# philcn/DXRExperiments

Measured on AMD Instinct MI355X. Metric: Mrays/s (all traced rays: primary + secondary + shadow), 1080p 1 spp/frame progressive, rendered in deferred sets of 32 frames, higher is better.
Workload: dtype f32

## Files before the change

dxrexperiments_amd/csrc/rt_pipeline.hip:

```cpp
#include <hip/hip_fp16.h>

#include <array>
#include <new>
#include <utility>

#include "rt_shade.h"
#include "rt_pipeline_queues.h"

using namespace rtd;

namespace {

constexpr int CBLOCK = 1024;
RT_DEV void wave_add(uint32_t v, uint32_t *counter)
{
    for (int o = 32; o > 0; o >>= 1) v += (uint32_t)__shfl_xor((int)v, o, 64);
    if ((threadIdx.x & 63u) == 0u && v) atomicAdd(counter, v);
}


template <bool BATCH>
struct PrimarySrcT {
    const PipeDev &pd;
    RT_DEV uint32_t count() const { return pd.cap; }
    RT_DEV uint32_t flags() const { return RT_RAY_FLAG_CULL_BACK_FACING_TRIANGLES; }
    RT_DEV bool load(uint32_t q, RayD &r) const
    {
        uint32_t px, py;
        if (BATCH && pd.n_frames > 1u) {
            uint32_t ql;
            const uint32_t f = (uint32_t)__builtin_amdgcn_readfirstlane((int)slot_frame(pd, q, ql));
            const bool valid = pix_xy(pd, ql, px, py);
            r = primary_ray(pd, pd.pfcs[f].cameraParams, px, py);
            return valid;
        }
        const bool valid = pix_xy(pd, q, px, py);
        r = primary_ray(pd, px, py);
        return valid;
    }
    RT_DEV void overflow(uint32_t q) const
    {
        const uint32_t k = atomicAdd(&pd.retry[0], 1u);
        if (k < pd.retry_cap) pd.retry[2u + k] = q;
    }
};
typedef PrimarySrcT<true> PrimarySrc;
struct PrimaryRetrySrc {
    const PipeDev &pd;
    RT_DEV uint32_t count() const { const uint32_t n = pd.retry[0]; return n <= pd.retry_cap ? n : pd.cap; }
    RT_DEV uint32_t flags() const { return RT_RAY_FLAG_CULL_BACK_FACING_TRIANGLES; }
    RT_DEV bool load(uint32_t i, RayD &r, uint32_t &ticket) const
    {
        const uint32_t q = pd.retry[0] <= pd.retry_cap ? pd.retry[2u + i] : i;
        ticket = q;
        uint32_t px, py, ql;
        const uint32_t f = slot_frame(pd, q, ql);
        const bool valid = pix_xy(pd, ql, px, py);
        r = pd.n_frames > 1u ? primary_ray(pd, pd.pfcs[f].cameraParams, px, py) : primary_ray(pd, px, py);
        return valid;
    }
};
template <bool BATCH>
struct PrimarySinkT {
    const PipeDev &pd;
    RT_DEV void store(uint32_t q, const HitD &h, bool) const
    {
        const bool hit = h.inst != RT_NO_HIT;
        pd.lv[0].hit[q] = make_float4(hit ? h.t : HIT_MISS, h.u, h.v, __uint_as_float(h.prim));
        pd.lv[0].inst[q] = h.inst;
    }
};

#ifndef RT_WAVES_PER_EU
#define RT_WAVES_PER_EU __attribute__((amdgpu_waves_per_eu(TWO_LEVEL ? 5 : RT_ROWS(STACK) == RT_LDS_STACK_ROWS_SETS ? 7 : RT_ROWS(STACK) == RT_LDS_STACK_ROWS ? 6 : 1)))
#endif
template <int STACK, bool TWO_LEVEL, bool BATCH, bool PERSIST>
__global__ void __launch_bounds__(PBLOCK) RT_WAVES_PER_EU k_primary(PipeDev pd)
{
    __shared__ int smem[(RT_ROWS(STACK) + RT_TOP_ROWS(PBLOCK)) * PBLOCK];
    if (blockIdx.x == 0)
        for (uint32_t i = threadIdx.x; i < (uint32_t)(POOL_OFFSET_WORDS + POOL_BYTES / 4); i += PBLOCK) pd.counters[i] = 0u;
    PrimarySrcT<BATCH> src = {pd};
    PrimarySinkT<BATCH> sink = {pd};
    if (PERSIST) trace_wave<RT_ROWS(STACK), PBLOCK, TWO_LEVEL, 64u, false, false, false, RT_REFS(STACK)>(pd.sc, src, sink, pd.pools + POOL_BYTES / 4, smem, nullptr);
    else trace_wave<RT_ROWS(STACK), PBLOCK, TWO_LEVEL, 64u, false, false, true, RT_REFS(STACK)>(pd.sc, src, sink, nullptr, smem, nullptr);
}

template <int STACK, bool TWO_LEVEL>
__global__ void __launch_bounds__(PBLOCK) RT_WAVES_PER_EU k_primary_retry(PipeDev pd)
{
    __shared__ int smem[(RT_ROWS(STACK) + RT_TOP_ROWS(PBLOCK)) * PBLOCK];
    if (pd.retry[0] == 0u) return;
    PrimaryRetrySrc src = {pd};
    PrimarySinkT<true> sink = {pd};
    trace_wave<RT_ROWS(STACK), PBLOCK, TWO_LEVEL, 64u, false, false, false, RT_REFS(STACK)>(pd.sc, src, sink, nullptr, smem, nullptr);
}

constexpr int CTILES = 8;
__global__ void __launch_bounds__(CBLOCK) k_compact_level(PipeDev pd, int L)
{
    __shared__ uint32_t wave_total[CBLOCK / 64];
    __shared__ uint32_t block_base;
    uint32_t total_items, n = 0;
    if (L == 0) total_items = pd.cap;
    else { n = pd.counters[C_NHIT + L - 1]; total_items = (L == 1 ? 2u : 1u) * n; }
    if (L == 0 && pd.retry && blockIdx.x == 0 && threadIdx.x == 0) { pd.retry[1] = pd.retry[0]; pd.retry[0] = 0u; }
    const uint32_t first = blockIdx.x * (uint32_t)(CTILES * CBLOCK);
    if (first >= total_items) return;
    const uint32_t lane = threadIdx.x & 63u, wave = threadIdx.x >> 6;
    auto slot_of = [&](uint32_t idx) -> size_t { return L == 1 ? (size_t)(idx / n) * pd.lv[1].rstride + idx % n : (size_t)idx; };
    uint32_t flags = 0, mine = 0;
#pragma unroll 4
    for (int t = 0; t < CTILES; t++) {
        const uint32_t idx = first + (uint32_t)t * CBLOCK + threadIdx.x;
        const bool hit = idx < total_items && pd.lv[L].hit[slot_of(idx)].x >= 0.0f;
        flags |= (hit ? 1u : 0u) << t;
        mine += hit ? 1u : 0u;
    }
    for (int o = 32; o > 0; o >>= 1) mine += (uint32_t)__shfl_xor((int)mine, o, 64);
    if (lane == 0) wave_total[wave] = mine;
    __syncthreads();
    if (threadIdx.x == 0) {
        uint32_t sum = 0;
        for (int w = 0; w < CBLOCK / 64; w++) sum += wave_total[w];
        block_base = sum ? atomicAdd(&pd.counters[C_NHIT + L], sum) : 0u;
    }
    __syncthreads();
    uint32_t running = block_base;
    for (int t = 0; t < CTILES; t++) {
        const uint32_t idx = first + (uint32_t)t * CBLOCK + threadIdx.x;
        if (first + (uint32_t)t * CBLOCK >= total_items) break;
        const bool hit = (flags >> t) & 1u;
        const unsigned long long mask = __ballot(hit);
        __syncthreads();
        if (lane == 0) wave_total[wave] = (uint32_t)__popcll(mask);
        __syncthreads();
        uint32_t before = 0, tile_total = 0;
        for (int w = 0; w < CBLOCK / 64; w++) { const uint32_t c = wave_total[w]; before += w < (int)wave ? c : 0u; tile_total += c; }
        const uint32_t j = running + before + (uint32_t)__popcll(mask & ((1ull << lane) - 1ull));
        if (idx < total_items) {
            const size_t slot = slot_of(idx);
            pd.lv[L].slot_j[slot] = hit ? j : RT_NO_HIT;
            if (hit) pd.lv[L].jlist[j] = (uint32_t)slot;
        }
        running += tile_total;
    }
}

template <bool PRIMARY, bool BATCH, int LC>
RT_DEV void shade_emit_body(const PipeDev &pd_arg, int level, uint32_t shadow_slots, uint32_t emit_next)
{
    PipeDev pd = pd_arg;
    const int L = PRIMARY ? 0 : (LC >= 0 ? LC : level);
    __builtin_assume(PRIMARY || L >= 1);
    const uint32_t idx = blockIdx.x * PBLOCK + threadIdx.x;
    if (idx >= pd.counters[C_NHIT + L]) return;
    const uint32_t slot = pd.lv[L].jlist[idx];
    const uint32_t q = L == 0 ? slot : pd.lv[L].pix[slot];
    uint32_t px, py, ql = q, frame = 0;
    if (BATCH) { frame = slot_frame(pd, q, ql); pd.pfc = pd.pfcs[frame]; }
    (void)pix_xy(pd, ql, px, py);
    const RayD r = L == 0 ? primary_ray(pd, px, py) : load_ray(pd.lv[L].O, pd.lv[L].D, slot);
    const float4 h = pd.lv[L].hit[slot];
    if (!PRIMARY && !emit_next && pd.shadow_compact && !pd.skip_unlit) {
        const f3 P = r.o + r.d * h.x;
        uint32_t mask = 3u;
        if (pd.kind != RT_PIPELINE_REALTIME && pd.pfc.options.debug == 2) {
            uint32_t seed = init_rand(px + py * pd.width, pd.pfc.cameraParams.frameCount);
            mask = next_rand(seed) < 0.5f ? 1u : 2u;
        }
        if ((uint32_t)L < pd.sh_levels) pd.sh_hits[pd.sh_cbase[L] + idx] = make_float4(P.x, P.y, P.z, __uint_as_float(mask | (frame << 8)));
        return;
    }
    EmitIO io(pd, L, idx, q, frame);
    (void)closest_hit(pd, io, r, h.x, h.y, h.z, __float_as_uint(h.w), pd.lv[L].inst[slot], (uint32_t)L, px + py * pd.width);
    io.finish_shadows(shadow_slots);
    if (emit_next) {
        if (L == 0) {
            for (uint32_t w = 0; w < 2; w++)
                if (!(io.sec_mask & (1u << w))) store_invalid(pd.lv[1].O, pd.lv[1].D, (size_t)w * pd.lv[1].rstride + idx);
        } else if (L < MAXD && !io.sec_mask) store_invalid(pd.lv[L < MAXD ? L + 1 : MAXD].O, pd.lv[L < MAXD ? L + 1 : MAXD].D, idx);
    }
}
template <bool PRIMARY, bool BATCH>
__global__ void __launch_bounds__(PBLOCK) k_shade_emit(PipeDev pd, int level, uint32_t shadow_slots, uint32_t emit_next)
{
    if (PRIMARY || !BATCH) shade_emit_body<PRIMARY, BATCH, -1>(pd, level, shadow_slots, emit_next);
    else if (level == 1) shade_emit_body<PRIMARY, BATCH, 1>(pd, level, shadow_slots, emit_next);
    else if (level == 2) shade_emit_body<PRIMARY, BATCH, 2>(pd, level, shadow_slots, emit_next);
    else if (level == 3) shade_emit_body<PRIMARY, BATCH, 3>(pd, level, shadow_slots, emit_next);
    else shade_emit_body<PRIMARY, BATCH, MAXD>(pd, level, shadow_slots, emit_next);
}

struct QueueSrc {
    const float4 *O, *D;
    const uint32_t *count_ptr;
    uint32_t stride, batches, fl;
    RT_DEV uint32_t n() const { return *count_ptr; }
    RT_DEV uint32_t count() const { return n() * batches; }
    RT_DEV uint32_t flags() const { return fl; }
    RT_DEV size_t slot(uint32_t i) const
    {
        const uint32_t c = n(), b = i >= c ? 1u : 0u;
        return (size_t)b * stride + (i - b * c);
    }
    RT_DEV bool load(uint32_t i, RayD &r) const
    {
        const size_t sl = slot(i);
        const v4f a = ldg16(O, sl * 16), b = ldg16(D, sl * 16);
        r.o = mk3(a.x, a.y, a.z); r.tmin = a.w;
        r.d = mk3(b.x, b.y, b.z); r.tmax = b.w;
        return r.tmax > r.tmin;
    }
};
struct SecondarySink {
    QueueSrc q;
    float4 *hit1;
    uint32_t *inst1;
    RT_DEV void store(uint32_t i, const HitD &h, bool traced) const
    {
        const size_t sl = q.slot(i);
        const bool hit = h.inst != RT_NO_HIT;
        hit1[sl] = make_float4(hit ? h.t : (traced ? HIT_MISS : HIT_UNTRACED), h.u, h.v, __uint_as_float(h.prim));
        inst1[sl] = h.inst;
    }
};

struct ShadowQueue {
    const float4 *hits, *O, *D;
    uint32_t *vis;
    const uint32_t *nhit;
    uint32_t log2, fl;
    uint32_t lv_first, lv_count;
    uint32_t cbase[MAXD + 1], hstride[MAXD + 1];
    LightRays lights;
    const LightRays *frame_lights;
    ShadowCacheDev cache;
    RT_DEV uint32_t count() const
    {
        uint32_t b = 0;
#pragma unroll
        for (uint32_t k = 0; k <= (uint32_t)MAXD; k++) if (k >= lv_first && k < lv_first + lv_count) b += (nhit[k] + 63u) & ~63u;
        return b << log2;
    }
    RT_DEV uint32_t flags() const { return fl; }
};
template <bool BATCH>
struct ShadowSrcN : ShadowQueue {
    RT_DEV bool load(uint32_t i, RayD &r, uint32_t &ticket) const
    {
        uint32_t n = 0, R = 0, cb = 0, hs = 0, before = 0;
        ticket = 0;
#pragma unroll
        for (uint32_t k = 0; k <= (uint32_t)MAXD; k++) {
            if (k >= lv_first && k < lv_first + lv_count) {
                const uint32_t nk = nhit[k], Rk = (nk + 63u) & ~63u, start = before;
                before += Rk << log2;
                const bool here = i >= start;
                n = here ? nk : n; R = here ? Rk : R; cb = here ? cbase[k] : cb; hs = here ? hstride[k] : hs;
                if (here) ticket = start;
            }
        }
        const uint32_t local = i - ticket;
        uint32_t b = local >= R ? 1u : 0u;
        if (log2 > 1u) { b += local >= 2u * R ? 1u : 0u; b += local >= 3u * R ? 1u : 0u; }
        const uint32_t j = local - b * R;
        ticket = (cb << log2) + b * hs + j;
        r.o = mk3(0.0f, 0.0f, 0.0f);
        r.d = mk3(0.0f, 0.0f, 0.0f);
        r.tmin = 0.0f;
        r.tmax = -1.0f;
        if (j >= n) { ticket = RT_NO_HIT; return false; }
        if (lights.on) {
            const v4f a = ldg16(hits, (size_t)(cb + j) * 16);
            const uint32_t bits = __float_as_uint(a.w);
            r.o = mk3(a.x, a.y, a.z);
            if (!((bits >> b) & 1u)) return false;
            if ((bits >> (2u + b)) & 1u) { r.tmax = RT_TMAX_SKIPPED; return false; }
            r.tmin = RAY_EPSILON;
            const LightRays *per_frame = BATCH ? frame_lights : nullptr;
            if (per_frame) {
                const float *fl = b == 0u ? per_frame[(bits >> 8) & 0xffu].dir_to_light : per_frame[(bits >> 8) & 0xffu].point_pos;
                const f3 l = mk3(fl[0], fl[1], fl[2]);
                if (b == 0u) { r.d = l; r.tmax = RAY_MAX_T; }
                else {
                    const f3 path = l - r.o;
                    const float dist = length(path);
                    r.d = normalize(path);
                    r.tmax = dist - fmaxf(RAY_EPSILON, fl[3]);
                }
                return r.tmax > r.tmin;
            }
            if (b == 0u) {
                r.d = mk3(lights.dir_to_light[0], lights.dir_to_light[1], lights.dir_to_light[2]);
                r.tmax = RAY_MAX_T;
            } else {
                const f3 path = mk3(lights.point_pos[0], lights.point_pos[1], lights.point_pos[2]) - r.o;
                const float dist = length(path);
                r.d = normalize(path);
                r.tmax = dist - fmaxf(RAY_EPSILON, lights.point_free);
            }
            return r.tmax > r.tmin;
        }
        const v4f a = ldg16(O, (size_t)ticket * 16), d = ldg16(D, (size_t)ticket * 16);
        r.o = mk3(a.x, a.y, a.z); r.tmin = a.w;
        r.d = mk3(d.x, d.y, d.z); r.tmax = d.w;
        return r.tmax > r.tmin;
    }
    RT_DEV uint32_t cache_slot(const RayD &r) const
    {
        const uint32_t res = cache.res;
        if (!(r.tmax < 1.0e37f)) {
            float u = r.o.x * cache.ua[0] + r.o.y * cache.ua[1] + r.o.z * cache.ua[2] + cache.ua[3];
            float v = r.o.x * cache.va[0] + r.o.y * cache.va[1] + r.o.z * cache.va[2] + cache.va[3];
            u = fminf(fmaxf(u, 0.0f), cache.res_f - 1.0f);
            v = fminf(fmaxf(v, 0.0f), cache.res_f - 1.0f);
            return (uint32_t)u * res + (uint32_t)v;
        }
        const float mx = r.o.x - cache.lp[0], my = r.o.y - cache.lp[1], mz = r.o.z - cache.lp[2];
        const float ax = fabsf(mx), ay = fabsf(my), az = fabsf(mz);
        uint32_t face;
        float ma, s, t;
        if (ax >= ay && ax >= az) { face = mx < 0.0f ? 1u : 0u; ma = ax; s = my; t = mz; }
        else if (ay >= az) { face = my < 0.0f ? 3u : 2u; ma = ay; s = mz; t = mx; }
        else { face = mz < 0.0f ? 5u : 4u; ma = az; s = mx; t = my; }
        const float inv = __builtin_amdgcn_rcpf(ma), half = 0.5f * cache.res_f;
        const float cs = fminf(fmaxf((s * inv * 0.5f + 0.5f) * half, 0.0f), half - 1.0f);
        const float ct = fminf(fmaxf((t * inv * 0.5f + 0.5f) * half, 0.0f), half - 1.0f);
        const uint32_t r2 = res >> 1;
        return res * res + (face * r2 + (uint32_t)cs) * r2 + (uint32_t)ct;
    }
    static constexpr bool has_first_candidates = true;
    template <bool TWO_LEVEL>
    RT_DEV uint32_t cached_leaf(uint32_t ticket, const RayD &r, uint32_t &slot, uint32_t &instance) const
    {
        slot = RT_NO_HIT;
        instance = 0u;
        if (!cache.table) return RT_NO_HIT;
        slot = RT_NO_HIT;
        if (cache.px_base && ticket < 2u * cache.hstride0) {
            const uint32_t b = ticket >= cache.hstride0 ? 1u : 0u;
            uint32_t q = cache.jlist0[ticket - b * cache.hstride0];
            if (cache.n_frames > 1u) q = (__umulhi(q >> 6, cache.frames_magic) << 6) | (q & 63u);
            if (q < cache.px_slots) slot = cache.px_base + 2u * q + b;
        }
        if (slot == RT_NO_HIT) slot = cache_slot(r);
        if (TWO_LEVEL) {
            const uint2 e = ((const uint2 *)cache.table)[slot];
            instance = e.y;
            return e.x;
        }
        const uint32_t t = cache.table[slot];
        return t < cache.n_tris ? t : RT_NO_HIT;
    }
    template <bool TWO_LEVEL>
    RT_DEV void remember(uint32_t slot, uint32_t sorted_triangle, uint32_t instance) const
    {
        if (!cache.table || slot >= cache.entries) return;
        if (TWO_LEVEL) ((uint2 *)cache.table)[slot] = make_uint2(sorted_triangle, instance);
        else cache.table[slot] = sorted_triangle;
    }
};
struct ShadowSinkN {
    ShadowQueue s;
    RT_DEV void store(uint32_t ticket, const HitD &h, bool) const { if (ticket != RT_NO_HIT && h.inst == RT_NO_HIT) atomicOr(&s.vis[ticket >> 5], 1u << (ticket & 31u)); }
};

template <int STACK, bool TWO_LEVEL, bool BATCH>
__global__ void __launch_bounds__(PBLOCK) RT_WAVES_PER_EU k_trace_shadow(SceneDev sc, ShadowQueue queues, uint32_t *pool, uint32_t *stat)
{
    __shared__ int smem[(RT_ROWS(STACK) + RT_TOP_ROWS(PBLOCK)) * PBLOCK];
    ShadowSrcN<BATCH> src;
    static_cast<ShadowQueue &>(src) = queues;
    ShadowSinkN sink = {queues};
    trace_wave<RT_ROWS(STACK), PBLOCK, TWO_LEVEL, (!TWO_LEVEL && RT_ROWS(STACK) == RT_LDS_STACK_ROWS_SETS) ? RT_POOL_CHUNK_SETS_ANYHIT : RT_POOL_CHUNK, RT_SHADOW_UNORDERED != 0, false, false, RT_REFS(STACK)>(sc, src, sink, pool, smem, stat);
}

template <int STACK, bool TWO_LEVEL>
__global__ void __launch_bounds__(PBLOCK) RT_WAVES_PER_EU k_trace_secondary(SceneDev sc, QueueSrc src, float4 *hit1, uint32_t *inst1, uint32_t *pool, uint32_t *stat)
{
    __shared__ int smem[(RT_ROWS(STACK) + RT_TOP_ROWS(PBLOCK)) * PBLOCK];
    SecondarySink sink = {src, hit1, inst1};
    trace_wave<RT_ROWS(STACK), PBLOCK, TWO_LEVEL, (!TWO_LEVEL && RT_ROWS(STACK) == RT_LDS_STACK_ROWS_SETS) ? RT_POOL_CHUNK_SETS : RT_POOL_CHUNK, false, false, false, RT_REFS(STACK)>(sc, src, sink, pool, smem, stat);
}

struct NullSink { RT_DEV void store(uint32_t, const HitD &, bool) const {} };

template <bool TWO_LEVEL>
__global__ void __launch_bounds__(PBLOCK) k_walk_primary(PipeDev pd, unsigned long long *walk)
{
    __shared__ int smem[(RT_LDS_STACK_ROWS + RT_TOP_ROWS(PBLOCK)) * PBLOCK];
    PrimarySrc src = {pd};
    NullSink sink;
    trace_wave<RT_LDS_STACK_ROWS, PBLOCK, TWO_LEVEL, 64u, false, true, false, true>(pd.sc, src, sink, nullptr, smem, nullptr, walk);
}
template <bool TWO_LEVEL>
__global__ void __launch_bounds__(PBLOCK) k_walk_queue(SceneDev sc, QueueSrc src, unsigned long long *walk)
{
    __shared__ int smem[(RT_LDS_STACK_ROWS + RT_TOP_ROWS(PBLOCK)) * PBLOCK];
    NullSink sink;
    trace_wave<RT_LDS_STACK_ROWS, PBLOCK, TWO_LEVEL, RT_POOL_CHUNK, false, true, false, true>(sc, src, sink, nullptr, smem, nullptr, walk);
}
template <bool TWO_LEVEL>
__global__ void __launch_bounds__(PBLOCK) k_walk_shadow(SceneDev sc, ShadowQueue queue, unsigned long long *walk)
{
    __shared__ int smem[(RT_LDS_STACK_ROWS + RT_TOP_ROWS(PBLOCK)) * PBLOCK];
    ShadowSrcN<true> src;
    static_cast<ShadowQueue &>(src) = queue;
    NullSink sink;
    trace_wave<RT_LDS_STACK_ROWS, PBLOCK, TWO_LEVEL, RT_POOL_CHUNK, RT_SHADOW_UNORDERED != 0, true, false, true>(sc, src, sink, nullptr, smem, nullptr, walk);
}

RT_DEV void add_totals(const uint32_t *__restrict__ counters, unsigned long long *__restrict__ totals, uint32_t pixels, uint32_t frames)
{
    totals[0] += (unsigned long long)pixels * frames;
    totals[1] += counters[C_SECONDARY];
    totals[2] += counters[C_SHADOW] + counters[C_SHADOW_SKIPPED];
    totals[6] += counters[C_SHADOW_SKIPPED];
    totals[3] += counters[C_NHIT + 0];
    for (int l = 1; l <= MAXD; l++) totals[4] += counters[C_NHIT + l];
    totals[5] += frames;
}

RT_DEV float4 accumulate(const PipeDev &pd, const float4 prev, const Shaded &sh)
{
    const f3 c = sh.color;
    const float4 cur = make_float4(fmax2(c.x, 0.0f), fmax2(c.y, 0.0f), fmax2(c.z, 0.0f), 1.0f);
    if (pd.accum_mode == RT_ACCUM_SUM) return make_float4(prev.x + cur.x, prev.y + cur.y, prev.z + cur.z, prev.w + cur.w);
    const float n = (float)pd.pfc.cameraParams.accumCount;
    const float n1 = (float)(pd.pfc.cameraParams.accumCount + 1u);
    float4 m = make_float4((n * prev.x + cur.x) / n1, (n * prev.y + cur.y) / n1, (n * prev.z + cur.z) / n1, (n * prev.w + cur.w) / n1);
    if (pd.accum_f16 == 1u) m = make_float4(__half2float(__float2half_rn(m.x)), __half2float(__float2half_rn(m.y)), __half2float(__float2half_rn(m.z)), __half2float(__float2half_rn(m.w)));
    else if (pd.accum_f16 == 2u) m = make_float4(__half2float(__float2half_rz(m.x)), __half2float(__float2half_rz(m.y)), __half2float(__float2half_rz(m.z)), __half2float(__float2half_rz(m.w)));
    return m;
}
RT_DEV void write_aovs(const PipeDev &pd, size_t pixel, const Shaded &sh)
{
    pd.aov_direct[pixel] = make_float4(fmax2(sh.aov_direct.x, 0.0f), fmax2(sh.aov_direct.y, 0.0f), fmax2(sh.aov_direct.z, 0.0f), 1.0f);
    pd.aov_indirect[pixel] = make_float4(fmax2(sh.aov_indirect.x, 0.0f), fmax2(sh.aov_indirect.y, 0.0f), fmax2(sh.aov_indirect.z, 0.0f), 1.0f);
}

template <bool FLAT, bool BATCH>
__global__ void __launch_bounds__(PBLOCK) k_resolve(PipeDev pd_arg)
{
    PipeDev pd = pd_arg;
    const uint32_t ql = blockIdx.x * PBLOCK + threadIdx.x;
    if (ql == 0) add_totals(pd.counters, pd.totals, pd.n_pixels, pd.n_frames);
    if (ql >= pd.fcap) return;
    uint32_t px, py;
    if (!pix_xy(pd, ql, px, py)) return;
    const size_t pixel = (size_t)py * pd.width + px;
    const bool progressive = pd.kind != RT_PIPELINE_REALTIME;
#ifndef RT_RESOLVE_REG_ACC
#define RT_RESOLVE_REG_ACC 1
#endif
    constexpr bool KEEP = BATCH && !FLAT && RT_RESOLVE_REG_ACC;
    float4 acc = KEEP && progressive ? pd.accum[pixel] : make_float4(0.0f, 0.0f, 0.0f, 0.0f);
    for (uint32_t f = 0; f < (BATCH ? pd.n_frames : 1u); f++) {
        if (BATCH) pd.pfc = pd.pfcs[f];
        const uint32_t q = frame_slot(pd, f, ql);
        const RayD r = primary_ray(pd, px, py);
        const float4 h = pd.lv[0].hit[q];
        Shaded sh;
        if (h.x == HIT_MISS) {
            sh.color = sample_environment(pd, r.d);
            sh.aov_direct = sh.color;
            sh.aov_indirect = mk3(0.0f, 0.0f, 0.0f);
        } else if (FLAT) {
            LevelResolveIO io(pd, 0, pd.lv[0].slot_j[q]);
            sh = closest_hit_aov(pd, io, r, h.x, h.y, h.z, __float_as_uint(h.w), pd.lv[0].inst[q], 0u, px + py * pd.width);
        } else {
            ResolveIO<0, 1> io(pd, pd.lv[0].slot_j[q], px + py * pd.width);
            sh = closest_hit_aov(pd, io, r, h.x, h.y, h.z, __float_as_uint(h.w), pd.lv[0].inst[q], 0u, px + py * pd.width);
        }
        if (progressive) { acc = accumulate(pd, KEEP ? acc : pd.accum[pixel], sh); if (!KEEP) pd.accum[pixel] = acc; }
        else write_aovs(pd, pixel, sh);
    }
    if (KEEP && progressive) pd.accum[pixel] = acc;
}

template <bool BATCH, int LC>
RT_DEV void shade_level_body(const PipeDev &pd_arg, int level)
{
    PipeDev pd = pd_arg;
    const int L = LC >= 0 ? LC : level;
    const uint32_t idx = blockIdx.x * PBLOCK + threadIdx.x;
    if (idx >= pd.counters[C_NHIT + L]) return;
    const uint32_t slot = pd.lv[L].jlist[idx];
    const uint32_t q = pd.lv[L].pix[slot];
    uint32_t px, py, ql = q;
    if (BATCH) pd.pfc = pd.pfcs[slot_frame(pd, q, ql)];
    (void)pix_xy(pd, ql, px, py);
    const RayD r = load_ray(pd.lv[L].O, pd.lv[L].D, slot);
    const float4 h = pd.lv[L].hit[slot];
    LevelResolveIO io(pd, L, idx);
    const f3 c = closest_hit(pd, io, r, h.x, h.y, h.z, __float_as_uint(h.w), pd.lv[L].inst[slot], (uint32_t)L, px + py * pd.width);
    pd.lv[L].color[slot] = make_float4(c.x, c.y, c.z, 0.0f);
}
template <bool BATCH>
__global__ void __launch_bounds__(PBLOCK) k_shade_level(PipeDev pd, int L)
{
    if (!BATCH) shade_level_body<BATCH, -1>(pd, L);
    else if (L == 1) shade_level_body<BATCH, 1>(pd, L);
    else if (L == 2) shade_level_body<BATCH, 2>(pd, L);
    else if (L == 3) shade_level_body<BATCH, 3>(pd, L);
    else shade_level_body<BATCH, MAXD>(pd, L);
}

RT_DEV void wave_add64(unsigned long long v, unsigned long long *counter)
{
    for (int o = 32; o > 0; o >>= 1) v += (unsigned long long)__shfl_xor((long long)v, o, 64);
    if ((threadIdx.x & 63u) == 0u && v) atomicAdd(counter, v);
}

template <class Src>
__global__ void __launch_bounds__(PBLOCK)
k_count_queue(SceneDev sc, Src src, unsigned long long *__restrict__ out)
{
    const uint32_t idx = blockIdx.x * PBLOCK + threadIdx.x;
    unsigned long long rays = 0, nodes = 0, tris = 0;
    if (idx < src.count()) {
        RayD r;
        uint32_t ticket;
        if (load_ray_of(src, idx, r, ticket, 0)) {
            uint32_t cn, ct;
            (void)trace_canonical(sc, r, src.flags(), cn, ct);
            rays = 1; nodes = cn; tris = ct;
        }
    }
    wave_add64(rays, &out[0]);
    wave_add64(nodes, &out[1]);
    wave_add64(tris, &out[2]);
}

__global__ void __launch_bounds__(PBLOCK) k_count_primary(PipeDev pd, unsigned long long *__restrict__ out)
{
    const uint32_t q = blockIdx.x * PBLOCK + threadIdx.x;
    unsigned long long rays = 0, nodes = 0, tris = 0;
    RayD r;
    const PrimarySrc src = {pd};
    if (q < pd.cap && src.load(q, r)) {
        uint32_t cn, ct;
        (void)trace_canonical(pd.sc, r, RT_RAY_FLAG_CULL_BACK_FACING_TRIANGLES, cn, ct);
        rays = 1; nodes = cn; tris = ct;
    }
    wave_add64(rays, &out[0]);
    wave_add64(nodes, &out[1]);
    wave_add64(tris, &out[2]);
}

__global__ void k_debug_cube(PipeDev pd, const float *__restrict__ dirs, float *__restrict__ out, size_t n)
{
    const size_t i = (size_t)blockIdx.x * blockDim.x + threadIdx.x;
    if (i >= n) return;
    const f3 c = sample_cube(pd, mk3(dirs[3 * i], dirs[3 * i + 1], dirs[3 * i + 2]));
    out[3 * i] = c.x; out[3 * i + 1] = c.y; out[3 * i + 2] = c.z;
}


}

namespace {

template <int STACK, bool TWO_LEVEL>
int launch_frame(rt_pipeline *p, PipeDev &pd, uint32_t shadow_slots, bool counted)
{
    hipError_t first_error = hipSuccess;
    auto record = [&](hipEvent_t e, hipStream_t s) { const hipError_t rc = hipEventRecord(e, s); if (first_error == hipSuccess) first_error = rc; };
    hipStream_t st = p->ctx->stream;
    const bool T = p->ring_frames > 0;
    const size_t ring_slot = T ? (size_t)(p->ring_pos % (uint64_t)p->ring_frames) : 0;
    hipEvent_t *ev = T ? &p->ring[ring_slot * EV_COUNT] : nullptr;
    const uint32_t cap = pd.cap;
    rt_context *ctx = p->ctx;
    const uint32_t levels = frame_levels(p);
    const bool deep = levels > 1, compact = pd.shadow_compact != 0;
    const uint32_t any = RT_RAY_FLAG_ACCEPT_FIRST_HIT_AND_END_SEARCH | RT_RAY_FLAG_SKIP_CLOSEST_HIT_SHADER;
    size_t hits_l = cap, slots = cap;
    size_t sh_total = 0;
    auto size_next = [&](uint32_t l, bool casts_shadows, bool spawns) -> int {
        if (counted) {
            HIP_TRY(hipMemcpyAsync(ctx->pinned, &pd.counters[C_NHIT + l], 4, hipMemcpyDeviceToHost, st));
            HIP_TRY(hipStreamSynchronize(st));
            hits_l = round64((size_t)ctx->pinned[0]);
            if (hits_l == 0) hits_l = 64;
        } else hits_l = l == 0 ? (size_t)cap : 2 * (size_t)cap;
        if (hits_l > 0xffffffc0ull / 2) { rt_set_error("render: more than 2^31 hits at radiance level %u", l); return RT_ERR_UNSUPPORTED; }
        pd.lv[l].hstride = (uint32_t)hits_l;
        if (casts_shadows) {
            if (((sh_total + hits_l) << pd.sh_log2) >= 0xffffffc0ull) { rt_set_error("render: more than 2^32 shadow rays in one set of launches"); return RT_ERR_UNSUPPORTED; }
            if (counted) RT_TRY(reserve_shadows(p, sh_total + hits_l, pd.sh_log2, compact, sh_total));
            pd.sh_cbase[l] = (uint32_t)sh_total;
            sh_total += hits_l;
        }
        bind_level(p, pd, (int)l);
        if (spawns) {
            slots = (l == 0 ? 2 : 1) * hits_l;
            if (l == 0) pd.lv[1].rstride = (uint32_t)hits_l;
            if (counted) RT_TRY(reserve_level_rays(p, l + 1, slots, deep));
            bind_level(p, pd, (int)l + 1);
        }
        return RT_OK;
    };
    if (T) record(ev[0], st);
    if (pd.primary_persistent) HIP_TRY(hipMemsetAsync(pd.pools + POOL_BYTES / 4, 0, PRIMARY_POOL_WORDS * 4, st));
    if (pd.primary_persistent) {
        if (pd.n_frames > 1u) k_primary<STACK, TWO_LEVEL, true, true><<<rt_persistent_grid(ctx, k_primary<STACK, TWO_LEVEL, true, true>, PBLOCK, cap), PBLOCK, 0, st>>>(pd);
        else k_primary<STACK, TWO_LEVEL, false, true><<<rt_persistent_grid(ctx, k_primary<STACK, TWO_LEVEL, false, true>, PBLOCK, cap), PBLOCK, 0, st>>>(pd);
    } else {
        if (pd.n_frames > 1u) k_primary<STACK, TWO_LEVEL, true, false><<<blocks(cap), PBLOCK, 0, st>>>(pd);
        else k_primary<STACK, TWO_LEVEL, false, false><<<blocks(cap), PBLOCK, 0, st>>>(pd);
        if (pd.retry) k_primary_retry<STACK, TWO_LEVEL><<<rt_persistent_grid(ctx, k_primary_retry<STACK, TWO_LEVEL>, PBLOCK, cap), PBLOCK, 0, st>>>(pd);
    }
    k_compact_level<<<(cap + CTILES * CBLOCK - 1) / (CTILES * CBLOCK), CBLOCK, 0, st>>>(pd, 0);
    if (T) record(ev[1], st);
    RT_TRY(size_next(0, true, levels >= 1));
    const bool B = pd.n_frames > 1u;
    if (B) k_shade_emit<true, true><<<blocks(hits_l), PBLOCK, 0, st>>>(pd, 0, shadow_slots, levels >= 1 ? 1u : 0u);
    else k_shade_emit<true, false><<<blocks(hits_l), PBLOCK, 0, st>>>(pd, 0, shadow_slots, levels >= 1 ? 1u : 0u);
    if (T) record(ev[2], st);
    const LightRays lr = light_rays(pd);
    for (uint32_t l = 1; l <= levels; l++) {
        const QueueSrc rays = {pd.lv[l].O, pd.lv[l].D, &pd.counters[C_NHIT + l - 1], pd.lv[1].rstride, l == 1 ? 2u : 1u, RT_RAY_FLAG_NONE};
        k_trace_secondary<STACK, TWO_LEVEL><<<rt_persistent_grid(ctx, k_trace_secondary<STACK, TWO_LEVEL>, PBLOCK, slots), PBLOCK, 0, st>>>(
            pd.sc, rays, pd.lv[l].hit, pd.lv[l].inst, pd.pools + (size_t)l * RT_POOL_GROUPS * RT_POOL_STRIDE, &pd.counters[C_SECONDARY]);
        k_compact_level<<<(unsigned)((slots + CTILES * CBLOCK - 1) / (CTILES * CBLOCK)), CBLOCK, 0, st>>>(pd, (int)l);
        if (T) record(ev[3 + 2 * (l - 1)], st);
        const bool casts_shadows = l < pd.sh_levels, spawns = l < levels;
        RT_TRY(size_next(l, casts_shadows, spawns));
        if (casts_shadows || spawns) {
            if (B) k_shade_emit<false, true><<<blocks(hits_l), PBLOCK, 0, st>>>(pd, (int)l, 2u, spawns ? 1u : 0u);
            else k_shade_emit<false, false><<<blocks(hits_l), PBLOCK, 0, st>>>(pd, (int)l, 2u, spawns ? 1u : 0u);
        }
        if (T) record(ev[4 + 2 * (l - 1)], st);
    }
    {
        ShadowQueue sq;
        memset(&sq, 0, sizeof sq);
        sq.hits = pd.sh_hits; sq.O = pd.sh_O; sq.D = pd.sh_D; sq.vis = pd.sh_vis;
        sq.nhit = &pd.counters[C_NHIT];
        sq.log2 = pd.sh_log2; sq.fl = any;
        sq.lv_first = 0; sq.lv_count = pd.sh_levels;
        for (int k = 0; k <= MAXD; k++) { sq.cbase[k] = pd.sh_cbase[k]; sq.hstride[k] = pd.lv[k].hstride; }
        sq.lights = lr;
        sq.frame_lights = B ? pd.frame_lights : nullptr;
        sq.cache = p->shadow_cache_dev;
        sq.cache.jlist0 = pd.lv[0].jlist;
        sq.cache.hstride0 = pd.lv[0].hstride;
        sq.cache.n_frames = pd.n_frames;
        sq.cache.frames_magic = (uint32_t)(0x100000000ull / (pd.n_frames ? pd.n_frames : 1u)) + 1u;
        if (sq.cache.px_slots > pd.fcap) sq.cache.px_slots = pd.fcap;
        const size_t rays_max = sh_total << pd.sh_log2;
        HIP_TRY(hipMemsetAsync(pd.sh_vis, 0, ((rays_max + 31) / 32) * 4, st));
        if (B) k_trace_shadow<STACK, TWO_LEVEL, true><<<rt_persistent_grid(ctx, k_trace_shadow<STACK, TWO_LEVEL, true>, PBLOCK, rays_max), PBLOCK, 0, st>>>(
            pd.sc, sq, pd.pools, &pd.counters[C_SHADOW]);
        else k_trace_shadow<STACK, TWO_LEVEL, false><<<rt_persistent_grid(ctx, k_trace_shadow<STACK, TWO_LEVEL, false>, PBLOCK, rays_max), PBLOCK, 0, st>>>(
            pd.sc, sq, pd.pools, &pd.counters[C_SHADOW]);
    }
    if (T) record(ev[EV_SHADOW], st);
    if (levels <= 1) {
        if (B) k_resolve<false, true><<<blocks(pd.fcap), PBLOCK, 0, st>>>(pd);
        else k_resolve<false, false><<<blocks(pd.fcap), PBLOCK, 0, st>>>(pd);
    } else {
        for (uint32_t l = levels; l >= 1; l--) {
            const size_t n_l = pd.lv[l].hstride;
            if (B) k_shade_level<true><<<blocks(n_l), PBLOCK, 0, st>>>(pd, (int)l);
            else k_shade_level<false><<<blocks(n_l), PBLOCK, 0, st>>>(pd, (int)l);
        }
        if (B) k_resolve<true, true><<<blocks(pd.fcap), PBLOCK, 0, st>>>(pd);
        else k_resolve<true, false><<<blocks(pd.fcap), PBLOCK, 0, st>>>(pd);
    }
    if (T) { record(ev[EV_RESOLVE], st); p->ring_levels[ring_slot] = (uint8_t)levels; p->ring_nframes[ring_slot] = (uint8_t)pd.n_frames; p->ring_pos++; }
    HIP_TRY(first_error);
    return RT_OK;
}

template <int STACK>
int launch_frame_any(rt_pipeline *p, PipeDev &pd, uint32_t shadow_slots, bool counted)
{
    if (p->scene->has_refs)
        return p->scene->two_level ? launch_frame<STACK + RT_STACK_REFS, true>(p, pd, shadow_slots, counted) : launch_frame<STACK + RT_STACK_REFS, false>(p, pd, shadow_slots, counted);
    return p->scene->two_level ? launch_frame<STACK, true>(p, pd, shadow_slots, counted) : launch_frame<STACK, false>(p, pd, shadow_slots, counted);
}

template <bool TWO_LEVEL>
static int count_walk_launch(rt_pipeline *p, unsigned long long *w)
{
    hipStream_t st = p->ctx->stream;
    const rt_context *ctx = p->ctx;
    const PipeDev &pd = p->last_pd;
    const uint32_t cap = pd.cap;
    const uint32_t any = RT_RAY_FLAG_ACCEPT_FIRST_HIT_AND_END_SEARCH | RT_RAY_FLAG_SKIP_CLOSEST_HIT_SHADER;
    k_walk_primary<TWO_LEVEL><<<rt_persistent_grid(ctx, k_walk_primary<TWO_LEVEL>, PBLOCK, cap), PBLOCK, 0, st>>>(pd, w + RT_WALK_WORDS * RT_STAGE_PRIMARY);
    const unsigned gq = rt_persistent_grid(ctx, k_walk_queue<TWO_LEVEL>, PBLOCK, (size_t)cap * 2);
    const unsigned gs = rt_persistent_grid(ctx, k_walk_shadow<TWO_LEVEL>, PBLOCK, (size_t)cap * 2);
    ShadowQueue sq;
    memset(&sq, 0, sizeof sq);
    sq.hits = pd.sh_hits; sq.O = pd.sh_O; sq.D = pd.sh_D; sq.vis = pd.sh_vis;
    sq.nhit = &pd.counters[C_NHIT];
    sq.log2 = pd.sh_log2; sq.fl = any;
    sq.lights = light_rays(pd);
    sq.frame_lights = pd.n_frames > 1u ? pd.frame_lights : nullptr;
    for (int k = 0; k <= MAXD; k++) { sq.cbase[k] = pd.sh_cbase[k]; sq.hstride[k] = pd.lv[k].hstride; }
    sq.lv_first = 0; sq.lv_count = 1;
    k_walk_shadow<TWO_LEVEL><<<gs, PBLOCK, 0, st>>>(pd.sc, sq, w + RT_WALK_WORDS * RT_STAGE_SHADOW0);
    const uint32_t levels = pd.max_rad < (uint32_t)MAXD ? pd.max_rad : (uint32_t)MAXD;
    for (uint32_t l = 1; l <= levels; l++)
        k_walk_queue<TWO_LEVEL><<<gq, PBLOCK, 0, st>>>(pd.sc, QueueSrc{pd.lv[l].O, pd.lv[l].D, &pd.counters[C_NHIT + l - 1], pd.lv[1].rstride, l == 1 ? 2u : 1u, RT_RAY_FLAG_NONE},
                                                       w + RT_WALK_WORDS * RT_STAGE_SECONDARY);
    if (pd.sh_levels > 1u) {
        sq.lv_first = 1; sq.lv_count = pd.sh_levels - 1u;
        k_walk_shadow<TWO_LEVEL><<<gs, PBLOCK, 0, st>>>(pd.sc, sq, w + RT_WALK_WORDS * RT_STAGE_SHADOW1);
    }
    HIP_TRY(hipGetLastError());
    return RT_OK;
}

}

int rt_frame_launch(rt_pipeline *p, PipeDev &pd, uint32_t shadow_slots, bool counted, bool set_rows)
{
    if (p->ctx->lds_stack_rows == RT_LDS_STACK_ROWS_TEST) return launch_frame_any<RT_LDS_STACK_ROWS_TEST>(p, pd, shadow_slots, counted);
    if (set_rows) return launch_frame<RT_LDS_STACK_ROWS_SETS, false>(p, pd, shadow_slots, counted);
    return launch_frame_any<RT_LDS_STACK_ROWS>(p, pd, shadow_slots, counted);
}

int rt_frame_count_walk(rt_pipeline *p, unsigned long long *w)
{
    return p->scene->two_level ? count_walk_launch<true>(p, w) : count_walk_launch<false>(p, w);
}

int rt_frame_count_work(rt_pipeline *p, unsigned long long *w)
{
    hipStream_t st = p->ctx->stream;
    const PipeDev &pd = p->last_pd;
    const uint32_t cap = pd.cap;
    const uint32_t any = RT_RAY_FLAG_ACCEPT_FIRST_HIT_AND_END_SEARCH | RT_RAY_FLAG_SKIP_CLOSEST_HIT_SHADER;
    k_count_primary<<<blocks(cap), PBLOCK, 0, st>>>(pd, w + 3 * RT_STAGE_PRIMARY);
    ShadowSrcN<true> sq;
    memset(&sq, 0, sizeof sq);
    sq.hits = pd.sh_hits; sq.O = pd.sh_O; sq.D = pd.sh_D; sq.vis = pd.sh_vis;
    sq.nhit = &pd.counters[C_NHIT];
    sq.log2 = pd.sh_log2; sq.fl = any;
    sq.lights = light_rays(pd);
    sq.frame_lights = pd.n_frames > 1u ? pd.frame_lights : nullptr;
    for (int k = 0; k <= MAXD; k++) { sq.cbase[k] = pd.sh_cbase[k]; sq.hstride[k] = pd.lv[k].hstride; }
    sq.lv_first = 0; sq.lv_count = 1;
    k_count_queue<<<blocks((size_t)pd.lv[0].hstride << pd.sh_log2), PBLOCK, 0, st>>>(pd.sc, sq, w + 3 * RT_STAGE_SHADOW0);
    const uint32_t levels = pd.max_rad < (uint32_t)MAXD ? pd.max_rad : (uint32_t)MAXD;
    size_t deeper = 0;
    for (uint32_t l = 1; l <= levels; l++) {
        const uint32_t batches = l == 1 ? 2u : 1u;
        const size_t slots = l == 1 ? 2 * (size_t)pd.lv[1].rstride : (size_t)pd.lv[l - 1].hstride;
        k_count_queue<<<blocks(slots), PBLOCK, 0, st>>>(pd.sc, QueueSrc{pd.lv[l].O, pd.lv[l].D, &pd.counters[C_NHIT + l - 1], pd.lv[1].rstride, batches, RT_RAY_FLAG_NONE},
                                                        w + 3 * RT_STAGE_SECONDARY);
        if (l < pd.sh_levels) deeper += pd.lv[l].hstride;
    }
    if (pd.sh_levels > 1u) {
        sq.lv_first = 1; sq.lv_count = pd.sh_levels - 1u;
        k_count_queue<<<blocks(deeper << pd.sh_log2), PBLOCK, 0, st>>>(pd.sc, sq, w + 3 * RT_STAGE_SHADOW1);
    }
    HIP_TRY(hipGetLastError());
    return RT_OK;
}

int rt_frame_debug_cube(hipStream_t st, const PipeDev &pd, const float *dirs, float *out, size_t n)
{
    k_debug_cube<<<blocks(n), PBLOCK, 0, st>>>(pd, dirs, out, n);
    HIP_TRY(hipGetLastError());
    return RT_OK;
}
```

dxrexperiments_amd/csrc/rt_pipeline_dev.h:

```cpp
#pragma once

#include "rt_trace_wave.h"

namespace rtp {

using namespace rtd;


constexpr int PBLOCK = 256;
#ifndef RT_SHADOW_UNORDERED
#define RT_SHADOW_UNORDERED 1
#endif
static_assert(RT_SHADOW_UNORDERED != 0, "the shadow stage counts skipped slots in the ANYHIT walk only");

#define RAY_MAX_T 1.0e+38f
#define RAY_EPSILON 0.0001f
#define HLSL_PI 3.1415927f

#define HIT_MISS -1.0f
#define HIT_UNTRACED -2.0f

constexpr int MAXD = 4;
enum { C_NHIT = 0,
       C_SECONDARY = MAXD + 1, C_SHADOW = MAXD + 2,
       C_SHADOW_SKIPPED = MAXD + 3,
       C_COUNT = MAXD + 4 };

struct LevelDev {
    uint32_t rstride;
    uint32_t hstride;
    float4 *O, *D;
    float4 *hit; uint32_t *inst;
    uint32_t *slot_j, *jlist;
    uint32_t *pix;
    float4 *color;
};

struct LightRays {
    uint32_t on;
    float dir_to_light[3];
    float point_pos[3];
    float point_free;
};

struct ShadowCacheDev {
    uint32_t *table;
    float ua[4], va[4];
    float lp[3];
    float res_f;
    uint32_t res;
    uint32_t two_level;
    uint32_t n_tris;
    uint32_t px_base, entries;
    const uint32_t *jlist0;
    uint32_t hstride0;
    uint32_t n_frames, frames_magic;
    uint32_t px_slots;
};

#define RT_MAX_BATCH 32u

struct PipeDev {
    SceneDev sc;
    rt_per_frame_constants pfc;
    uint32_t n_frames, fcap;
    const rt_per_frame_constants *pfcs;
    const LightRays *frame_lights;
    const rt_material_params *mats;
    uint32_t nmats;
    const float4 *env;
    uint32_t env_size;
    uint32_t env_filter;
    float env_const[3];
    uint32_t width, height;
    uint32_t x0, y0, tw, th, cap;
    uint32_t tiles_x;
    uint32_t band_rows, band_rank, band_world;
    uint32_t n_pixels;
    uint32_t max_rad, max_shadow;
    uint32_t accum_mode;
    uint32_t accum_f16;
    uint32_t skip_unlit;
    uint32_t shadow_compact;
    uint32_t kind;
    uint32_t primary_persistent;
    float4 *accum;
    float4 *aov_direct, *aov_indirect;
    uint32_t *counters;
    uint32_t *retry;
    uint32_t retry_cap;
    unsigned long long *totals;
    float point_free;
    float4 *sh_hits, *sh_O, *sh_D;
    uint32_t *sh_vis;
    uint32_t sh_log2;
    uint32_t sh_levels;
    uint32_t sh_cbase[MAXD + 1];
    uint32_t *pools;
    LevelDev lv[MAXD + 1];
};

constexpr size_t POOL_BYTES = (size_t)(1 + MAXD) * RT_POOL_GROUPS * RT_POOL_STRIDE * 4;
constexpr size_t PRIMARY_POOL_WORDS = (size_t)RT_POOL_GROUPS * RT_POOL_STRIDE;
constexpr size_t POOL_OFFSET_WORDS = 64;

RT_DEV size_t sh_ray(const PipeDev &pd, int L, uint32_t idx, uint32_t s)
{
    return ((size_t)pd.sh_cbase[L] << pd.sh_log2) + (size_t)s * pd.lv[L].hstride + idx;
}
RT_DEV uint32_t shadow_bit(const PipeDev &pd, size_t n)
{
    return (pd.sh_vis[n >> 5] >> (uint32_t)(n & 31u)) & 1u;
}

inline unsigned blocks(size_t n) { return (unsigned)((n + PBLOCK - 1) / PBLOCK); }

}

using namespace rtp;


struct rt_pipeline {
    rt_context *ctx = nullptr;
    uint32_t kind = RT_PIPELINE_PROGRESSIVE;
    DevBuf aov_own;
    rt_scene *scene = nullptr;
    std::vector<rt_material_params> mats;
    DevBuf d_mats;
    bool mats_dirty = true;
    DevBuf d_env;
    uint32_t env_size = 0;
    uint32_t env_filter = RT_CUBE_SEAMLESS;
    float env_const[3] = {0.5f, 0.5f, 0.5f};
    uint32_t width = 0, height = 0, format = RT_FORMAT_R32G32B32A32_FLOAT;
    DevBuf accum_own;
    float4 *accum = nullptr;
    rt_per_frame_constants pfc;
    bool have_pfc = false;
    uint32_t max_rad = 1, max_shadow = 2, accum_mode = RT_ACCUM_RUNNING_MEAN, accum_f16 = 0;
    uint32_t skip_unlit = 0;
    size_t queue_budget = 0;
    bool counted_queues = false;
    uint32_t deferred_max = 0;
    std::vector<rt_per_frame_constants> pending;
    int deferred_error = RT_OK;
    std::string deferred_error_msg;
    struct LevelBuf { DevBuf O, D, hit, inst, slot_j, jlist, pix, color; } lv[MAXD + 1];
    DevBuf sh_hits, sh_O, sh_D, sh_vis;
    DevBuf counters;
    DevBuf retry;
    DevBuf half_out;
    std::vector<hipEvent_t> ring;
    std::vector<uint8_t> ring_levels;
    std::vector<uint8_t> ring_nframes;
    DevBuf batch_consts;
    int ring_frames = 0;
    DevBuf shadow_cache;
    int shadow_cache_res = -1;
    uint32_t shadow_cache_gen = 0xffffffffu;
    float shadow_cache_centre[3] = {0, 0, 0}, shadow_cache_radius = 1.0f;
    ShadowCacheDev shadow_cache_dev = {};
    struct FreeSphere {
        DevBuf d_min;
        float *h_min = nullptr;
        hipEvent_t landed = nullptr;
        uint32_t asked_gen = 0xffffffffu, known_gen = 0xffffffffu;
        float asked_lp[3] = {0, 0, 0}, known_lp[3] = {0, 0, 0}, known_radius = 0.0f;
        float asked_size = 0.0f;
        bool in_flight = false;
    } free_sphere;
    struct PrimaryMode {
        uint32_t *h_count = nullptr;
        hipEvent_t landed = nullptr;
        bool in_flight = false;
        uint32_t asked_slots = 0;
        uint32_t gen = 0xffffffffu;
        int samples = 0;
        bool persistent = false;
    } primary_mode;
    uint64_t ring_pos = 0;
    DevBuf totals, work;
    PipeDev last_pd;
    rt_stats stats;
    uint32_t last_tile[4] = {0, 0, 0, 0};
    uint32_t last_pixels = 0;
    bool rendered = false;
    uint32_t last_scene_gen = 0;
};

int rt_pipeline_flush_pending(rt_pipeline *p);

namespace rtp {


constexpr int EV_COUNT = 5 + 2 * MAXD;
constexpr int EV_SHADOW = 3 + 2 * MAXD, EV_RESOLVE = 4 + 2 * MAXD;

}
```

dxrexperiments_amd/csrc/rt_pipeline_render.hip:

```cpp
#include <hip/hip_fp16.h>

#include <array>
#include <new>
#include <utility>

#include "rt_pipeline_queues.h"

using namespace rtd;

namespace {

__global__ void __launch_bounds__(PBLOCK) k_free_sphere(SceneDev sc, uint32_t two_level, uint32_t n, float lx, float ly, float lz, uint32_t *out_bits)
{
    const uint32_t i = blockIdx.x * PBLOCK + threadIdx.x;
    float d2 = __uint_as_float(0x7f800000u);
    if (i < n) {
        float lo[3], hi[3];
        if (two_level) {
            const InstanceRec &in = sc.inst[i];
            for (int c = 0; c < 3; c++) { lo[c] = in.wlo[c]; hi[c] = in.whi[c]; }
        } else {
            const TriRec t = sc.inst[0].tris[i];
            const float vx[3] = {t.a.x, t.a.w, t.b.z}, vy[3] = {t.a.y, t.b.x, t.b.w}, vz[3] = {t.a.z, t.b.y, t.c.x};
            lo[0] = fminf(vx[0], fminf(vx[1], vx[2])); hi[0] = fmaxf(vx[0], fmaxf(vx[1], vx[2]));
            lo[1] = fminf(vy[0], fminf(vy[1], vy[2])); hi[1] = fmaxf(vy[0], fmaxf(vy[1], vy[2]));
            lo[2] = fminf(vz[0], fminf(vz[1], vz[2])); hi[2] = fmaxf(vz[0], fmaxf(vz[1], vz[2]));
        }
        const float l[3] = {lx, ly, lz};
        float s = 0.0f;
        bool known = true;
        for (int c = 0; c < 3; c++) {
            const float d = l[c] < lo[c] ? lo[c] - l[c] : l[c] > hi[c] ? l[c] - hi[c] : 0.0f;
            known = known && lo[c] == lo[c] && hi[c] == hi[c];
            s += d * d;
        }
        d2 = known ? s : 0.0f;
    }
    for (int o = 32; o > 0; o >>= 1) d2 = fminf(d2, __shfl_xor(d2, o, 64));
    if ((threadIdx.x & 63u) == 0u) atomicMin(out_bits, __float_as_uint(d2));
}

void free_sphere_poll(rt_pipeline::FreeSphere &f)
{
    if (f.in_flight && hipEventQuery(f.landed) == hipSuccess) {
        f.in_flight = false;
        f.known_gen = f.asked_gen;
        memcpy(f.known_lp, f.asked_lp, sizeof f.known_lp);
        double size = 0.0;
        for (int c = 0; c < 3; c++) size = fmax(size, fmax(fabs((double)f.asked_lp[c]), (double)f.asked_size));
        const double r = sqrt((double)*f.h_min) * 0.99 - (double)RAY_EPSILON - size * 4e-6;
        f.known_radius = r > 0.0 && r < 1e30 ? (float)r : 0.0f;
    }
}

float free_radius(rt_pipeline *p, const PipeDev &pd, const float lp[3])
{
    rt_pipeline::FreeSphere &f = p->free_sphere;
    const rt_scene *s = p->scene;
    hipStream_t st = p->ctx->stream;
    if (!(lp[0] == lp[0] && lp[1] == lp[1] && lp[2] == lp[2])) return 0.0f;
    if (!f.h_min) {
        if (hipHostMalloc((void **)&f.h_min, 64, hipHostMallocDefault) != hipSuccess) { f.h_min = nullptr; return 0.0f; }
        if (hipEventCreateWithFlags(&f.landed, hipEventDisableTiming) != hipSuccess || f.d_min.reserve(64) != RT_OK) return 0.0f;
    }
    free_sphere_poll(f);
    const bool known = f.known_gen == s->generation && memcmp(f.known_lp, lp, sizeof f.known_lp) == 0;
    const bool asked = f.in_flight && f.asked_gen == s->generation && memcmp(f.asked_lp, lp, sizeof f.asked_lp) == 0;
    if (!known && !asked && !f.in_flight) {
        const uint32_t n = s->two_level ? (uint32_t)s->inst.size() : (s->inst.empty() || !s->inst[0].model ? 0u : s->inst[0].model->n_recs);
        if (n == 0u || !f.landed) return 0.0f;
        if (hipMemsetD32Async((hipDeviceptr_t)f.d_min.p, 0x7f800000, 1, st) != hipSuccess) return 0.0f;
        k_free_sphere<<<(n + PBLOCK - 1) / PBLOCK, PBLOCK, 0, st>>>(pd.sc, s->two_level ? 1u : 0u, n, lp[0], lp[1], lp[2], f.d_min.as<uint32_t>());
        if (hipMemcpyAsync(f.h_min, f.d_min.p, 4, hipMemcpyDeviceToHost, st) != hipSuccess || hipEventRecord(f.landed, st) != hipSuccess) return 0.0f;
        f.in_flight = true;
        f.asked_gen = s->generation;
        const float *bb = s->two_level ? s->tlas.bounds : s->inst[0].model->blas.bounds;
        f.asked_size = 0.0f;
        for (int c = 0; c < 6; c++) f.asked_size = bb[c] == bb[c] ? fmaxf(f.asked_size, fabsf(bb[c])) : __builtin_inff();
        memcpy(f.asked_lp, lp, sizeof f.asked_lp);
    }
    return known ? f.known_radius : 0.0f;
}

int prepare_shadow_cache(rt_pipeline *p, const rt_per_frame_constants &pfc, const LightRays &lr)
{
    p->shadow_cache_dev = ShadowCacheDev{};
    const rt_scene *s = p->scene;
    if (p->shadow_cache_res == 0 || s->inst.empty()) return RT_OK;
    size_t n_tris_all = 0;
    for (const SceneInstance &si : s->inst) {
        if (!si.model || si.model->n_tris >= (1u << 28)) return RT_OK;
        n_tris_all += si.model->n_tris;
    }
    int want = p->shadow_cache_res;
    if (want < 0) {
        want = p->ctx->opt_shadow_cache_res;
        if (want == 0) return RT_OK;
    }
    if (want < 0) {
        const double target = 8.0 * sqrt((double)n_tris_all);
        want = 1024;
        while (want < 8192 && (double)want < target) want *= 2;
    }
    if (want > 8192) want = 8192;
    if (want < 16) want = 16;
    const uint32_t res = (uint32_t)want & ~1u;
    const int per_pixel_opt = p->ctx->opt_shadow_cache_pixels;
    const bool per_pixel = per_pixel_opt < 0 ? s->two_level : per_pixel_opt != 0;
    const size_t cells = (size_t)res * res + 6u * (size_t)(res / 2) * (res / 2);
    const size_t px_slots = per_pixel ? (size_t)((p->width + 7u) / 8u) * ((p->height + 7u) / 8u) * 64u : 0;
    const size_t entries = cells + 2 * px_slots, entry_bytes = s->two_level ? 8 : 4;
    if (entries >= 0xffffffffull) return RT_OK;
    if (p->shadow_cache.bytes < entries * entry_bytes) { RT_TRY(p->shadow_cache.reserve(entries * entry_bytes)); p->shadow_cache_gen = 0xffffffffu; }
    if (lr.on == 0xffffffffu) return RT_OK;
    if (p->shadow_cache_gen != s->generation) {
        HIP_TRY(hipMemsetAsync(p->shadow_cache.p, 0xff, entries * entry_bytes, p->ctx->stream));
        const float *bb = s->two_level ? s->tlas.bounds : s->inst[0].model->blas.bounds;
        float lo[3], hi[3];
        for (int c = 0; c < 3; c++) {
            lo[c] = bb[c]; hi[c] = bb[3 + c];
            if (!(lo[c] > -1e30f && hi[c] < 1e30f && lo[c] <= hi[c])) { lo[c] = -1.0f; hi[c] = 1.0f; }
        }
        float r2 = 0.0f;
        for (int c = 0; c < 3; c++) { p->shadow_cache_centre[c] = 0.5f * (lo[c] + hi[c]); const float h = 0.5f * (hi[c] - lo[c]); r2 += h * h; }
        p->shadow_cache_radius = r2 > 0.0f && r2 < 1e30f ? sqrtf(r2) : 1.0f;
        p->shadow_cache_gen = s->generation;
    }
    ShadowCacheDev c = {};
    c.table = p->shadow_cache.as<uint32_t>();
    c.res = res; c.res_f = (float)res;
    c.two_level = s->two_level ? 1u : 0u;
    c.n_tris = s->two_level ? 0u : s->inst[0].model->n_recs;
    c.entries = (uint32_t)entries;
    c.px_base = px_slots ? (uint32_t)cells : 0u;
    c.px_slots = (uint32_t)px_slots;
    const float d[3] = {lr.dir_to_light[0], lr.dir_to_light[1], lr.dir_to_light[2]};
    const float ref[3] = {fabsf(d[1]) < 0.9f ? 0.0f : 1.0f, fabsf(d[1]) < 0.9f ? 1.0f : 0.0f, 0.0f};
    float a[3] = {d[1] * ref[2] - d[2] * ref[1], d[2] * ref[0] - d[0] * ref[2], d[0] * ref[1] - d[1] * ref[0]};
    const float al = sqrtf(a[0] * a[0] + a[1] * a[1] + a[2] * a[2]);
    if (!(al > 1e-6f)) { a[0] = 1.0f; a[1] = 0.0f; a[2] = 0.0f; } else { a[0] /= al; a[1] /= al; a[2] /= al; }
    const float b[3] = {d[1] * a[2] - d[2] * a[1], d[2] * a[0] - d[0] * a[2], d[0] * a[1] - d[1] * a[0]};
    const float k = 0.5f * (float)res / p->shadow_cache_radius;
    c.ua[3] = 0.5f * (float)res; c.va[3] = 0.5f * (float)res;
    for (int i = 0; i < 3; i++) {
        c.ua[i] = a[i] * k; c.va[i] = b[i] * k;
        c.ua[3] -= p->shadow_cache_centre[i] * c.ua[i];
        c.va[3] -= p->shadow_cache_centre[i] * c.va[i];
        c.lp[i] = lr.point_pos[i];
    }
    (void)pfc;
    p->shadow_cache_dev = c;
    return RT_OK;
}

int scene_for_set(rt_pipeline *p, uint32_t n_frames, size_t cap, SceneDev *out, bool *sets_kernels = nullptr)
{
    rt_context *ctx = p->ctx;
    const bool seven_waves_always = ctx->opt_seven_waves_always;
    const bool set_rows = (n_frames > 1 || seven_waves_always) && !p->scene->two_level && !p->scene->has_refs && ctx->lds_stack_rows != RT_LDS_STACK_ROWS_TEST && RT_LDS_STACK_ROWS_SETS != RT_LDS_STACK_ROWS;
    const size_t resident = (size_t)ctx->cu_count * (ctx->blocks_per_cu_override > (uint32_t)RT_RESIDENT_BLOCKS_PER_CU ? ctx->blocks_per_cu_override : (uint32_t)RT_RESIDENT_BLOCKS_PER_CU) * PBLOCK;
    (void)cap;
    if (sets_kernels) *sets_kernels = set_rows;
    return rt_scene_dev_for_launch(ctx, p->scene, set_rows ? RT_LDS_STACK_ROWS_SETS : rt_lds_stack_rows(ctx), resident, out);
}

}

extern "C" {

static int render_region(rt_pipeline *p, uint32_t width, uint32_t height, uint32_t x0, uint32_t y0, uint32_t x1, uint32_t y1,
                         uint32_t band_rows, uint32_t band_rank, uint32_t band_world, const rt_per_frame_constants *frames = nullptr, uint32_t n_frames = 1)
{
    RT_REQUIRE(p, "null pipeline");
    if (!p->scene || !p->scene->built) { rt_set_error("render: acceleration structures not built"); return RT_ERR_STATE; }
    if (!p->accum) { rt_set_error("render: no output resource"); return RT_ERR_STATE; }
    if (!frames && !p->have_pfc) { rt_set_error("render: update() has not been called"); return RT_ERR_STATE; }
    if (!frames) { frames = &p->pfc; n_frames = 1; }
    RT_REQUIRE(n_frames >= 1 && n_frames <= RT_MAX_BATCH, "batch size");
    if (p->mats.empty()) { rt_set_error("render: no material"); return RT_ERR_STATE; }
    RT_REQUIRE(width == p->width && height == p->height, "width/height differ from the output resource");
    if (x1 > width) x1 = width;
    if (!band_rows && y1 > height) y1 = height;
    RT_REQUIRE(x0 < x1 && y0 < y1, "empty tile");
    rt_context *ctx = p->ctx;
    HIP_TRY(hipSetDevice(ctx->device));
    hipStream_t st = ctx->stream;
    p->rendered = false;
    if (p->kind == RT_PIPELINE_PROGRESSIVE && frames[0].cameraParams.accumCount >= frames[0].options.maxIterations) {
        memset(&p->stats, 0, sizeof p->stats);
        return RT_OK;
    }
    if (p->mats_dirty) {
        RT_TRY(p->d_mats.reserve(sizeof(rt_material_params) * p->mats.size()));
        HIP_TRY(hipMemcpyAsync(p->d_mats.p, p->mats.data(), sizeof(rt_material_params) * p->mats.size(), hipMemcpyHostToDevice, st));
        p->mats_dirty = false;
    }
    const uint32_t tw = x1 - x0, th = y1 - y0;
    const uint32_t tiles_x = (tw + 7u) / 8u, fcap = tiles_x * ((th + 7u) / 8u) * 64u;
    RT_REQUIRE((uint64_t)fcap * n_frames < 0x40000000ull, "batch: more than 2^30 pixel slots in one set of launches");
    const uint32_t cap = fcap * n_frames;
    const bool ao_view = p->kind == RT_PIPELINE_PROGRESSIVE && frames[0].options.showAmbientOcclusionOnly;
    const uint32_t shadow_slots = ao_view ? 4u : 2u;
    const uint32_t levels_now = frame_levels(p);
    const bool counted = worst_case_queue_bytes(cap, levels_now, p->max_shadow, shadow_slots, !ao_view) > queue_budget(p);
    if (p->counters.bytes < POOL_OFFSET_WORDS * 4 + POOL_BYTES + PRIMARY_POOL_WORDS * 4) {
        RT_TRY(p->counters.reserve(POOL_OFFSET_WORDS * 4 + POOL_BYTES + PRIMARY_POOL_WORDS * 4));
        HIP_TRY(hipMemsetAsync(p->counters.p, 0, p->counters.bytes, st));
    }
    if (counted) RT_TRY(reserve_level_rays(p, 0, cap, levels_now > 1));
    else RT_TRY(reserve_worst_case(p, cap, levels_now, p->max_shadow, shadow_slots, !ao_view));
    p->counted_queues = counted;
    if (!p->totals.p) {
        RT_TRY(p->totals.reserve(8 * sizeof(unsigned long long)));
        HIP_TRY(hipMemsetAsync(p->totals.p, 0, 8 * sizeof(unsigned long long), st));
    }
    PipeDev pd;
    bool set_rows = false;
    RT_TRY(scene_for_set(p, n_frames, cap, &pd.sc, &set_rows));
    pd.pfc = frames[0];
    pd.n_frames = n_frames; pd.fcap = fcap;
    pd.pfcs = nullptr; pd.frame_lights = nullptr;
    pd.shadow_compact = ao_view ? 0u : 1u;
    const bool free_on = ctx->opt_free_radius;
    {
        const float lp0[3] = {frames[0].pointLight.worldPos.x, frames[0].pointLight.worldPos.y, frames[0].pointLight.worldPos.z};
        pd.point_free = free_on ? free_radius(p, pd, lp0) : 0.0f;
    }
    if (ao_view) p->shadow_cache_dev = ShadowCacheDev{};
    else RT_TRY(prepare_shadow_cache(p, frames[0], light_rays(1u, frames[0])));
    if (n_frames > 1) {
        const size_t cb = sizeof(rt_per_frame_constants) * RT_MAX_BATCH, lb = sizeof(LightRays) * RT_MAX_BATCH;
        RT_TRY(p->batch_consts.reserve(cb + lb));
        std::vector<unsigned char> stage(cb + lb, 0);
        for (uint32_t f = 0; f < n_frames; f++) {
            memcpy(&stage[sizeof(rt_per_frame_constants) * f], &frames[f], sizeof(rt_per_frame_constants));
            LightRays lr = light_rays(pd.shadow_compact, frames[f]);
            lr.point_free = free_on && memcmp(lr.point_pos, &frames[0].pointLight.worldPos, 3 * sizeof(float)) == 0 ? pd.point_free : 0.0f;
            memcpy(&stage[cb + sizeof(LightRays) * f], &lr, sizeof lr);
        }
        HIP_TRY(hipMemcpyAsync(p->batch_consts.p, stage.data(), cb + lb, hipMemcpyHostToDevice, st));
        pd.pfcs = p->batch_consts.as<rt_per_frame_constants>();
        pd.frame_lights = (const LightRays *)((const char *)p->batch_consts.p + cb);
    }
    pd.mats = p->d_mats.as<rt_material_params>();
    pd.nmats = (uint32_t)p->mats.size();
    pd.env = p->d_env.as<float4>();
    pd.env_size = p->env_size;
    pd.env_filter = p->env_filter;
    for (int k = 0; k < 3; k++) pd.env_const[k] = p->env_const[k];
    pd.width = width; pd.height = height;
    pd.x0 = x0; pd.y0 = y0; pd.tw = tw; pd.th = th; pd.cap = cap; pd.tiles_x = tiles_x;
    pd.band_rows = band_rows; pd.band_rank = band_rank; pd.band_world = band_world;
    uint32_t owned_rows = th;
    if (band_rows) {
        owned_rows = 0;
        for (uint32_t b = band_rank; (uint64_t)b * band_rows < height; b += band_world)
            owned_rows += (uint64_t)(b + 1) * band_rows <= height ? band_rows : height - b * band_rows;
    }
    pd.n_pixels = tw * owned_rows;
    pd.max_rad = p->max_rad; pd.max_shadow = p->max_shadow;
    pd.sh_log2 = ao_view ? 2u : 1u;
    pd.sh_levels = shadow_levels(levels_now, p->max_shadow);
    for (int k = 0; k <= MAXD; k++) pd.sh_cbase[k] = 0;
    pd.accum_mode = p->accum_mode;
    pd.accum_f16 = p->accum_f16;
    pd.skip_unlit = p->skip_unlit;
    pd.kind = p->kind;
    {
        rt_pipeline::PrimaryMode &pm = p->primary_mode;
        if (pm.gen != p->scene->generation) { pm.gen = p->scene->generation; pm.samples = 0; pm.persistent = false; pm.in_flight = false; }
        if (pm.in_flight && hipEventQuery(pm.landed) == hipSuccess) {
            pm.in_flight = false;
            pm.samples++;
            if ((double)*pm.h_count > 0.002 * (double)pm.asked_slots) pm.persistent = true;
        }
        pd.primary_persistent = (ctx->opt_primary_persistent < 0 ? (p->scene->two_level || pm.persistent) : ctx->opt_primary_persistent != 0) ? 1u : 0u;
    }
    pd.retry = nullptr;
    pd.retry_cap = 0;
    if (pd.sc.deep_stack && !pd.primary_persistent) {
        const uint32_t want = ctx->opt_primary_retry_cap ? ctx->opt_primary_retry_cap : (1u << 20);
        if (p->retry.bytes < (2 + (size_t)want) * 4) {
            RT_TRY(p->retry.reserve((2 + (size_t)want) * 4));
            HIP_TRY(hipMemsetAsync(p->retry.p, 0, 8, st));
        }
        pd.retry = p->retry.as<uint32_t>();
        pd.retry_cap = want;
    }
    pd.accum = p->accum;
    pd.aov_direct = p->accum;
    pd.aov_indirect = p->aov_own.as<float4>();
    pd.counters = p->counters.as<uint32_t>();
    for (int l = 0; l <= MAXD; l++) {
        bind_level(p, pd, l);
        pd.lv[l].rstride = cap;
        pd.lv[l].hstride = l == 0 ? cap : 2u * cap;
    }
    static_assert(C_COUNT <= POOL_OFFSET_WORDS, "scalar counters overlap the chunk pools");
    pd.pools = pd.counters + POOL_OFFSET_WORDS;
    pd.totals = p->totals.as<unsigned long long>();
    RT_TRY(rt_frame_launch(p, pd, shadow_slots, counted, set_rows));
    HIP_TRY(hipGetLastError());
    if (pd.retry && !p->primary_mode.in_flight && p->primary_mode.samples < 8 && ctx->opt_primary_persistent < 0) {
        rt_pipeline::PrimaryMode &pm = p->primary_mode;
        if (!pm.h_count) {
            if (hipHostMalloc((void **)&pm.h_count, 64, hipHostMallocDefault) != hipSuccess) pm.h_count = nullptr;
            else if (hipEventCreateWithFlags(&pm.landed, hipEventDisableTiming) != hipSuccess) { (void)hipHostFree(pm.h_count); pm.h_count = nullptr; pm.landed = nullptr; }
        }
        if (pm.h_count && hipMemcpyAsync(pm.h_count, pd.retry + 1, 4, hipMemcpyDeviceToHost, st) == hipSuccess && hipEventRecord(pm.landed, st) == hipSuccess) {
            pm.in_flight = true;
            pm.asked_slots = cap;
        }
    }
    p->last_pd = pd;
    p->last_scene_gen = p->scene->generation;
    p->last_tile[0] = x0; p->last_tile[1] = y0; p->last_tile[2] = x1; p->last_tile[3] = y1;
    p->last_pixels = pd.n_pixels * n_frames;
    p->rendered = true;
    return RT_OK;
}

static int render_frames(rt_pipeline *p, uint32_t width, uint32_t height, const rt_per_frame_constants *constants, uint32_t n,
                         uint32_t band_rows, uint32_t band_rank, uint32_t band_world)
{
    uint32_t band_count = 0;
    if (band_rows) {
        RT_TRY(rt_tile_bands(height, band_rows, band_rank, band_world, nullptr, nullptr, 0, &band_count));
        if (band_count == 0) n = 0;
    }
    uint32_t batch_max = RT_MAX_BATCH;
    if (p->ctx->opt_batch_max >= 1 && p->ctx->opt_batch_max <= RT_MAX_BATCH) batch_max = p->ctx->opt_batch_max;
    std::vector<rt_per_frame_constants> run;
    auto flush = [&]() -> int {
        for (size_t at = 0; at < run.size();) {
            const size_t n_now = run.size() - at < batch_max ? run.size() - at : batch_max;
            const int rc = band_rows ? render_region(p, width, height, 0, 0, width, band_count * band_rows, band_rows, band_rank, band_world, run.data() + at, (uint32_t)n_now)
                                     : render_region(p, width, height, 0, 0, width, height, 0, 0, 1, run.data() + at, (uint32_t)n_now);
            if (rc == RT_ERR_OOM && n_now > 1) { batch_max = (uint32_t)(n_now / 2); continue; }
            if (rc != RT_OK) { run.clear(); return rc; }
            at += n_now;
        }
        run.clear();
        return RT_OK;
    };
    for (uint32_t i = 0; i < n; i++) {
        const rt_per_frame_constants &c = constants[i];
        if (c.cameraParams.accumCount >= c.options.maxIterations) continue;
        if (!run.empty() && (run.size() >= batch_max || (run[0].options.showAmbientOcclusionOnly != 0) != (c.options.showAmbientOcclusionOnly != 0))) RT_TRY(flush());
        run.push_back(c);
    }
    return flush();
}

}

static int flush_pending_now(rt_pipeline *p)
{
    if (p->pending.empty()) return RT_OK;
    std::vector<rt_per_frame_constants> frames;
    frames.swap(p->pending);
    std::vector<rt_pipeline *> &reg = p->ctx->deferred;
    for (size_t k = 0; k < reg.size(); k++) if (reg[k] == p) { reg.erase(reg.begin() + (long)k); break; }
    const rt_per_frame_constants keep = p->pfc;
    const int rc = render_frames(p, p->width, p->height, frames.data(), (uint32_t)frames.size(), 0, 0, 1);
    p->pfc = keep;
    return rc;
}

int rt_pipeline_flush_pending(rt_pipeline *p)
{
    if (!p) return RT_OK;
    if (p->deferred_error != RT_OK) {
        const int rc = p->deferred_error;
        rt_set_error("deferred frames were lost: %s", p->deferred_error_msg.c_str());
        p->deferred_error = RT_OK;
        p->deferred_error_msg.clear();
        return rc;
    }
    return flush_pending_now(p);
}

int rt_context_flush_deferred(rt_context *ctx)
{
    if (!ctx) return RT_OK;
    while (!ctx->deferred.empty()) {
        rt_pipeline *p = ctx->deferred.back();
        const int rc = flush_pending_now(p);
        if (rc != RT_OK && p->deferred_error == RT_OK) { p->deferred_error = rc; p->deferred_error_msg = rt_last_error(); }
    }
    return RT_OK;
}

extern "C" {

int rt_pipeline_flush(rt_pipeline *p)
{
    RT_REQUIRE(p, "null pipeline");
    return rt_pipeline_flush_pending(p);
}

int rt_pipeline_set_deferred(rt_pipeline *p, uint32_t max_frames)
{
    RT_REQUIRE(p, "null pipeline");
    RT_REQUIRE(max_frames <= RT_MAX_BATCH, "set_deferred: at most 32 frames share a set of launches");
    RT_REQUIRE(p->kind == RT_PIPELINE_PROGRESSIVE || max_frames <= 1, "set_deferred: only the progressive pipeline accumulates frames");
    RT_TRY(rt_pipeline_flush_pending(p));
    p->deferred_max = max_frames;
    return RT_OK;
}

int rt_pipeline_get_deferred(const rt_pipeline *p, uint32_t *max_frames, uint32_t *pending)
{
    RT_REQUIRE(p, "null pipeline");
    if (max_frames) *max_frames = p->deferred_max;
    if (pending) *pending = (uint32_t)p->pending.size();
    return RT_OK;
}

int rt_pipeline_render_tile(rt_pipeline *p, uint32_t width, uint32_t height, uint32_t x0, uint32_t y0, uint32_t x1, uint32_t y1)
{
    RT_TRY(rt_pipeline_flush_pending(p));
    return render_region(p, width, height, x0, y0, x1, y1, 0, 0, 1);
}

int rt_pipeline_render_bands(rt_pipeline *p, uint32_t width, uint32_t height, uint32_t band_rows, uint32_t rank, uint32_t world)
{
    RT_REQUIRE(world > 0 && rank < world, "rank outside [0, world)");
    RT_REQUIRE(band_rows > 0 && band_rows % 8 == 0, "band_rows must be a positive multiple of 8 (pixel slots are 8x8 tiles)");
    RT_TRY(rt_pipeline_flush_pending(p));
    uint32_t n = 0;
    RT_TRY(rt_tile_bands(height, band_rows, rank, world, nullptr, nullptr, 0, &n));
    if (n == 0) return RT_OK;
    return render_region(p, width, height, 0, 0, width, n * band_rows, band_rows, rank, world);
}

int rt_pipeline_render(rt_pipeline *p, uint32_t width, uint32_t height)
{
    RT_REQUIRE(p, "null pipeline");
    if (p->deferred_max > 1 && p->kind == RT_PIPELINE_PROGRESSIVE) {
        if (!p->scene || !p->scene->built) { rt_set_error("render: acceleration structures not built"); return RT_ERR_STATE; }
        if (!p->accum) { rt_set_error("render: no output resource"); return RT_ERR_STATE; }
        if (!p->have_pfc) { rt_set_error("render: update() has not been called"); return RT_ERR_STATE; }
        if (p->mats.empty()) { rt_set_error("render: no material"); return RT_ERR_STATE; }
        RT_REQUIRE(width == p->width && height == p->height, "width/height differ from the output resource");
        if (p->pending.empty()) p->ctx->deferred.push_back(p);
        p->pending.push_back(p->pfc);
        p->rendered = false;
        if (p->pending.size() >= p->deferred_max) return rt_pipeline_flush_pending(p);
        return RT_OK;
    }
    return rt_pipeline_render_tile(p, width, height, 0, 0, width, height);
}

int rt_pipeline_render_batch(rt_pipeline *p, uint32_t width, uint32_t height, const rt_per_frame_constants *constants, uint32_t n)
{
    RT_REQUIRE(p && (constants || n == 0), "null argument");
    RT_REQUIRE(p->kind == RT_PIPELINE_PROGRESSIVE, "render_batch: only the progressive pipeline accumulates frames");
    RT_TRY(rt_pipeline_flush_pending(p));
    RT_TRY(render_frames(p, width, height, constants, n, 0, 0, 1));
    if (n) { p->pfc = constants[n - 1]; p->have_pfc = true; }
    return RT_OK;
}

int rt_pipeline_render_bands_batch(rt_pipeline *p, uint32_t width, uint32_t height, uint32_t band_rows, uint32_t rank, uint32_t world,
                                   const rt_per_frame_constants *constants, uint32_t n)
{
    RT_REQUIRE(p && (constants || n == 0), "null argument");
    RT_REQUIRE(p->kind == RT_PIPELINE_PROGRESSIVE, "render_bands_batch: only the progressive pipeline accumulates frames");
    RT_REQUIRE(world > 0 && rank < world, "rank outside [0, world)");
    RT_REQUIRE(band_rows > 0 && band_rows % 8 == 0, "band_rows must be a positive multiple of 8 (pixel slots are 8x8 tiles)");
    RT_TRY(rt_pipeline_flush_pending(p));
    RT_TRY(render_frames(p, width, height, constants, n, band_rows, rank, world));
    if (n) { p->pfc = constants[n - 1]; p->have_pfc = true; }
    return RT_OK;
}

int rt_pipeline_set_queue_budget(rt_pipeline *p, size_t bytes)
{
    RT_REQUIRE(p, "null pipeline");
    p->queue_budget = bytes;
    return RT_OK;
}

int rt_pipeline_get_queue_memory(rt_pipeline *p, size_t *bytes_reserved, uint32_t *sized_by_count)
{
    RT_REQUIRE(p, "null pipeline");
    size_t total = p->counters.bytes + p->batch_consts.bytes + p->sh_hits.bytes + p->sh_O.bytes + p->sh_D.bytes + p->sh_vis.bytes;
    for (const rt_pipeline::LevelBuf &l : p->lv) {
        const DevBuf *lb[] = {&l.O, &l.D, &l.hit, &l.inst, &l.slot_j, &l.jlist, &l.pix, &l.color};
        for (const DevBuf *b : lb) total += b->bytes;
    }
    if (bytes_reserved) *bytes_reserved = total;
    if (sized_by_count) *sized_by_count = p->counted_queues ? 1u : 0u;
    return RT_OK;
}

int rt_pipeline_reserve_batch(rt_pipeline *p, uint32_t width, uint32_t height, uint32_t frames)
{
    RT_REQUIRE(p && width > 0 && height > 0 && frames >= 1 && frames <= RT_MAX_BATCH, "reserve_batch: bad argument");
    HIP_TRY(hipSetDevice(p->ctx->device));
    const uint32_t fcap = ((width + 7u) / 8u) * ((height + 7u) / 8u) * 64u;
    RT_REQUIRE((uint64_t)fcap * frames < 0x40000000ull, "batch: more than 2^30 pixel slots in one set of launches");
    const bool ao_view = p->have_pfc && p->pfc.options.showAmbientOcclusionOnly != 0;
    const uint32_t levels_now = frame_levels(p);
    const size_t cap = (size_t)fcap * frames;
    RT_TRY(rt_pipeline_flush_pending(p));
    p->rendered = false;
    if (p->counters.bytes < POOL_OFFSET_WORDS * 4 + POOL_BYTES + PRIMARY_POOL_WORDS * 4) {
        RT_TRY(p->counters.reserve(POOL_OFFSET_WORDS * 4 + POOL_BYTES + PRIMARY_POOL_WORDS * 4));
        HIP_TRY(hipMemsetAsync(p->counters.p, 0, p->counters.bytes, p->ctx->stream));
    }
    if (worst_case_queue_bytes(cap, levels_now, p->max_shadow, ao_view ? 4u : 2u, !ao_view) > queue_budget(p)) RT_TRY(reserve_level_rays(p, 0, cap, levels_now > 1));
    else RT_TRY(reserve_worst_case(p, cap, levels_now, p->max_shadow, ao_view ? 4u : 2u, !ao_view));
    if (frames > 1) RT_TRY(p->batch_consts.reserve((sizeof(rt_per_frame_constants) + sizeof(LightRays)) * RT_MAX_BATCH));
    if (p->scene && p->scene->built) {
        SceneDev sc;
        RT_TRY(scene_for_set(p, frames, cap, &sc));
        LightRays only_allocate = no_light_rays();
        only_allocate.on = 0xffffffffu;
        RT_TRY(prepare_shadow_cache(p, p->pfc, only_allocate));
        p->shadow_cache_dev = ShadowCacheDev{};
    }
    return RT_OK;
}

int rt_pipeline_get_free_sphere(rt_pipeline *p, float *radius)
{
    RT_REQUIRE(p && radius, "get_free_sphere: null argument");
    *radius = 0.0f;
    rt_pipeline::FreeSphere &f = p->free_sphere;
    if (!p->scene || !p->have_pfc || !f.landed) return RT_OK;
    HIP_TRY(hipSetDevice(p->ctx->device));
    free_sphere_poll(f);
    const float *lp = &p->pfc.pointLight.worldPos.x;
    if (f.known_gen == p->scene->generation && memcmp(f.known_lp, lp, sizeof f.known_lp) == 0) *radius = f.known_radius;
    return RT_OK;
}

int rt_pipeline_count_work(rt_pipeline *p, rt_stage_work *out)
{
    RT_REQUIRE(p && out, "null argument");
    RT_TRY(rt_pipeline_flush_pending(p));
    if (!p->rendered || !p->scene->built || p->scene->generation != p->last_scene_gen) { rt_set_error("count_work: nothing rendered since the last change of scene, materials or output"); return RT_ERR_STATE; }
    HIP_TRY(hipSetDevice(p->ctx->device));
    hipStream_t st = p->ctx->stream;
    RT_TRY(p->work.reserve(RT_STAGE_COUNT * RT_WALK_WORDS * sizeof(unsigned long long)));
    HIP_TRY(hipMemsetAsync(p->work.p, 0, RT_STAGE_COUNT * 3 * sizeof(unsigned long long), st));
    unsigned long long *w = p->work.as<unsigned long long>();
    RT_TRY(rt_frame_count_work(p, w));
    unsigned long long h[RT_STAGE_COUNT * 3];
    HIP_TRY(hipMemcpyAsync(h, w, sizeof h, hipMemcpyDeviceToHost, st));
    HIP_TRY(hipStreamSynchronize(st));
    for (int k = 0; k < RT_STAGE_COUNT; k++) { out[k].rays = h[3 * k]; out[k].nodes = h[3 * k + 1]; out[k].tris = h[3 * k + 2]; }
    return RT_OK;
}

int rt_pipeline_count_walk(rt_pipeline *p, rt_stage_walk *out)
{
    RT_REQUIRE(p && out, "null argument");
    RT_TRY(rt_pipeline_flush_pending(p));
    if (!p->rendered || !p->scene->built || p->scene->generation != p->last_scene_gen) { rt_set_error("count_walk: nothing rendered since the last change of scene, materials or output"); return RT_ERR_STATE; }
    HIP_TRY(hipSetDevice(p->ctx->device));
    hipStream_t st = p->ctx->stream;
    const size_t bytes = RT_STAGE_COUNT * RT_WALK_WORDS * sizeof(unsigned long long);
    RT_TRY(p->work.reserve(bytes));
    HIP_TRY(hipMemsetAsync(p->work.p, 0, bytes, st));
    unsigned long long *w = p->work.as<unsigned long long>();
    RT_TRY(rt_frame_count_walk(p, w));
    unsigned long long h[RT_STAGE_COUNT * RT_WALK_WORDS];
    HIP_TRY(hipMemcpyAsync(h, w, sizeof h, hipMemcpyDeviceToHost, st));
    HIP_TRY(hipStreamSynchronize(st));
    for (int k = 0; k < RT_STAGE_COUNT; k++) {
        const unsigned long long *hk = h + RT_WALK_WORDS * k;
        out[k].rays = hk[0]; out[k].nodes_global = hk[1]; out[k].nodes_lds = hk[2];
        out[k].tris = hk[3]; out[k].instance_entries = hk[4]; out[k].lines = hk[5];
        out[k].longest_walk = hk[6] >> 32;
        out[k].longest_walk_ray = (uint32_t)hk[6];
        out[k].wave_node_steps = hk[7]; out[k].wave_leaf_phases = hk[8]; out[k].wave_tri_steps = hk[9]; out[k].node_lines = hk[10];
    }
    return RT_OK;
}

int rt_debug_read_secondary_ray(rt_pipeline *p, uint32_t index, float origin_tmin[4], float dir_tmax[4])
{
    RT_REQUIRE(p && origin_tmin && dir_tmax, "null argument");
    RT_TRY(rt_pipeline_flush_pending(p));
    if (!p->rendered) { rt_set_error("nothing rendered yet"); return RT_ERR_STATE; }
    HIP_TRY(hipSetDevice(p->ctx->device));
    HIP_TRY(hipStreamSynchronize(p->ctx->stream));
    uint32_t n = 0;
    HIP_TRY(hipMemcpy(&n, p->last_pd.counters + C_NHIT, 4, hipMemcpyDeviceToHost));
    RT_REQUIRE(n > 0 && index < 2 * n, "ray index out of range");
    const size_t slot = (size_t)(index / n) * p->last_pd.lv[1].rstride + index % n;
    HIP_TRY(hipMemcpy(origin_tmin, p->last_pd.lv[1].O + slot, 16, hipMemcpyDeviceToHost));
    HIP_TRY(hipMemcpy(dir_tmax, p->last_pd.lv[1].D + slot, 16, hipMemcpyDeviceToHost));
    return RT_OK;
}

int rt_pipeline_read_primary_hits(rt_pipeline *p, float *t, uint32_t *prim, uint32_t *inst)
{
    RT_REQUIRE(p, "null pipeline");
    RT_TRY(rt_pipeline_flush_pending(p));
    if (!p->rendered) { rt_set_error("nothing rendered yet"); return RT_ERR_STATE; }
    HIP_TRY(hipSetDevice(p->ctx->device));
    HIP_TRY(hipStreamSynchronize(p->ctx->stream));
    const PipeDev &pd = p->last_pd;
    const size_t cap = pd.cap;
    std::vector<float4> h(cap);
    std::vector<uint32_t> hi(cap);
    HIP_TRY(hipMemcpy(h.data(), p->lv[0].hit.p, cap * 16, hipMemcpyDeviceToHost));
    HIP_TRY(hipMemcpy(hi.data(), p->lv[0].inst.p, cap * 4, hipMemcpyDeviceToHost));
    for (size_t q = 0; q < cap; q++) {
        const uint32_t tl = (uint32_t)(q >> 6), w = (uint32_t)(q & 63u);
        const uint32_t lx = (tl % pd.tiles_x) * 8u + (w & 7u), ly = (tl / pd.tiles_x) * 8u + (w >> 3);
        if (lx >= pd.tw || ly >= pd.th) continue;
        const size_t i = (size_t)ly * pd.tw + lx;
        if (t) t[i] = h[q].x;
        if (prim) memcpy(&prim[i], &h[q].w, 4);
        if (inst) inst[i] = hi[q];
    }
    return RT_OK;
}

int rt_debug_sample_cube(rt_context *ctx, const float *faces, uint32_t size, uint32_t filter, const float *dirs, float *out, size_t n)
{
    RT_REQUIRE(ctx && faces && dirs && out && size > 0, "bad argument");
    RT_REQUIRE(filter == RT_CUBE_SEAMLESS || filter == RT_CUBE_FACE_CLAMP, "unknown cube-map filter");
    if (n == 0) return RT_OK;
    HIP_TRY(hipSetDevice(ctx->device));
    DevBuf *sb = ctx->scratch;
    const size_t fb = (size_t)6 * size * size * 16;
    RT_TRY(sb[0].reserve(fb)); RT_TRY(sb[1].reserve(n * 12)); RT_TRY(sb[2].reserve(n * 12));
    HIP_TRY(hipMemcpyAsync(sb[0].p, faces, fb, hipMemcpyHostToDevice, ctx->stream));
    HIP_TRY(hipMemcpyAsync(sb[1].p, dirs, n * 12, hipMemcpyHostToDevice, ctx->stream));
    PipeDev pd;
    memset(&pd, 0, sizeof pd);
    pd.env = sb[0].as<float4>();
    pd.env_size = size;
    pd.env_filter = filter;
    RT_TRY(rt_frame_debug_cube(ctx->stream, pd, sb[1].as<float>(), sb[2].as<float>(), n));
    HIP_TRY(hipMemcpyAsync(out, sb[2].p, n * 12, hipMemcpyDeviceToHost, ctx->stream));
    HIP_TRY(hipStreamSynchronize(ctx->stream));
    return RT_OK;
}

}
```

dxrexperiments_amd/csrc/rt_shade.h:

```cpp
#pragma once

#include "rt_pipeline_dev.h"

namespace rtp {

__constant__ const unsigned char kCubeEdge[24] = {
    (4 << 3) | 3, (5 << 3) | 1, (2 << 3) | 7, (3 << 3) | 3,
    (5 << 3) | 3, (4 << 3) | 1, (2 << 3) | 1, (3 << 3) | 5,
    (1 << 3) | 0, (0 << 3) | 4, (5 << 3) | 4, (4 << 3) | 0,
    (1 << 3) | 6, (0 << 3) | 2, (4 << 3) | 2, (5 << 3) | 6,
    (1 << 3) | 3, (0 << 3) | 1, (2 << 3) | 2, (3 << 3) | 0,
    (0 << 3) | 3, (1 << 3) | 1, (2 << 3) | 4, (3 << 3) | 6};

RT_DEV bool cube_tap(const PipeDev &pd, int face, int x, int y, float4 &out)
{
    const int m = (int)pd.env_size - 1;
    const bool ox = x < 0 || x > m, oy = y < 0 || y > m;
    if (pd.env_filter == RT_CUBE_FACE_CLAMP) {
        x = min(max(x, 0), m); y = min(max(y, 0), m);
    } else if (ox && oy) {
        return false;
    } else if (ox || oy) {
        const int e = ox ? (x < 0 ? 0 : 1) : (y < 0 ? 2 : 3);
        const int k = ox ? y : x;
        const unsigned code = kCubeEdge[face * 4 + e];
        const int fixed = (code & 2u) ? m : 0, run = (code & 4u) ? m - k : k;
        face = (int)(code >> 3);
        x = (code & 1u) ? fixed : run;
        y = (code & 1u) ? run : fixed;
    }
    out = pd.env[((size_t)face * pd.env_size + (size_t)y) * pd.env_size + (size_t)x];
    return true;
}

RT_DEV f3 sample_cube(const PipeDev &pd, f3 d)
{
    if (pd.env_size == 0) return mk3(pd.env_const[0], pd.env_const[1], pd.env_const[2]);
    const float ax = __builtin_fabsf(d.x), ay = __builtin_fabsf(d.y), az = __builtin_fabsf(d.z);
    int face; float ma, sc, tc;
    if (ax >= ay && ax >= az) { face = d.x > 0.0f ? 0 : 1; ma = ax; sc = d.x > 0.0f ? -d.z : d.z; tc = -d.y; }
    else if (ay >= az) { face = d.y > 0.0f ? 2 : 3; ma = ay; sc = d.x; tc = d.y > 0.0f ? d.z : -d.z; }
    else { face = d.z > 0.0f ? 4 : 5; ma = az; sc = d.z > 0.0f ? d.x : -d.x; tc = -d.y; }
    if (!(ma > 0.0f) || !(ma < __uint_as_float(0x7f800000u))) return mk3(0.0f, 0.0f, 0.0f);
    const float u = (sc / ma + 1.0f) * 0.5f;
    const float v = (tc / ma + 1.0f) * 0.5f;
    const float n = (float)pd.env_size;
    const float fx = u * n - 0.5f, fy = v * n - 0.5f;
    const float x0f = __builtin_floorf(fx), y0f = __builtin_floorf(fy);
    const float wx = fx - x0f, wy = fy - y0f;
    const int x0 = (int)x0f, y0 = (int)y0f;
    float4 c[4];
    bool have[4];
    have[0] = cube_tap(pd, face, x0, y0, c[0]);
    have[1] = cube_tap(pd, face, x0 + 1, y0, c[1]);
    have[2] = cube_tap(pd, face, x0, y0 + 1, c[2]);
    have[3] = cube_tap(pd, face, x0 + 1, y0 + 1, c[3]);
    for (int k = 0; k < 4; k++) {
        if (have[k]) continue;
        float sx = 0.0f, sy = 0.0f, sz = 0.0f;
        for (int j = 0; j < 4; j++)
            if (j != k) { sx = sx + c[j].x; sy = sy + c[j].y; sz = sz + c[j].z; }
        c[k] = make_float4(sx / 3.0f, sy / 3.0f, sz / 3.0f, 1.0f);
    }
    const float4 c00 = c[0], c10 = c[1], c01 = c[2], c11 = c[3];
    const float tx = c00.x + (c10.x - c00.x) * wx, bx = c01.x + (c11.x - c01.x) * wx;
    const float ty = c00.y + (c10.y - c00.y) * wx, by = c01.y + (c11.y - c01.y) * wx;
    const float tz = c00.z + (c10.z - c00.z) * wx, bz = c01.z + (c11.z - c01.z) * wx;
    return mk3(tx + (bx - tx) * wy, ty + (by - ty) * wy, tz + (bz - tz) * wy);
}

RT_DEV f3 sample_environment(const PipeDev &pd, f3 dir)
{
    return sample_cube(pd, dir) * pd.pfc.options.environmentStrength;
}

RT_DEV bool pix_xy(const PipeDev &pd, uint32_t q, uint32_t &px, uint32_t &py)
{
    const uint32_t t = q >> 6, w = q & 63u;
    const uint32_t lx = (t % pd.tiles_x) * 8u + (w & 7u), ly = (t / pd.tiles_x) * 8u + (w >> 3);
    px = pd.x0 + lx;
    if (pd.band_rows) {
        py = ((ly / pd.band_rows) * pd.band_world + pd.band_rank) * pd.band_rows + ly % pd.band_rows;
        return lx < pd.tw && ly < pd.th && py < pd.height;
    }
    py = pd.y0 + ly;
    return lx < pd.tw && ly < pd.th;
}

RT_DEV RayD primary_ray(const PipeDev &pd, const rt_camera_params &cp, uint32_t px, uint32_t py)
{
    const float dx = ((float)px + 0.5f) / (float)pd.width * 2.0f - 1.0f;
    const float dy = ((float)py + 0.5f) / (float)pd.height * 2.0f - 1.0f;
    const float js = pd.kind == RT_PIPELINE_REALTIME ? 10.0f : 30.0f;
    const float jx = cp.jitters.x * js, jy = cp.jitters.y * js;
    RayD r;
    r.o = mk3(cp.worldEyePos.x + jx, cp.worldEyePos.y + jy, cp.worldEyePos.z + 0.0f);
    f3 dir = mk3(cp.U.x, cp.U.y, cp.U.z) * dx;
    dir = dir + mk3(cp.V.x, cp.V.y, cp.V.z) * (-dy);
    dir = dir + mk3(cp.W.x, cp.W.y, cp.W.z);
    r.d = normalize(dir);
    r.tmin = 0.0f;
    r.tmax = RAY_MAX_T;
    return r;
}
RT_DEV RayD primary_ray(const PipeDev &pd, uint32_t px, uint32_t py) { return primary_ray(pd, pd.pfc.cameraParams, px, py); }

RT_DEV uint32_t slot_frame(const PipeDev &pd, uint32_t q, uint32_t &q_in_frame)
{
    if (pd.n_frames <= 1u) { q_in_frame = q; return 0u; }
    const uint32_t c = q >> 6, tile = c / pd.n_frames, f = c - tile * pd.n_frames;
    q_in_frame = (tile << 6) | (q & 63u);
    return f;
}
RT_DEV uint32_t frame_slot(const PipeDev &pd, uint32_t frame, uint32_t q_in_frame)
{
    return pd.n_frames <= 1u ? q_in_frame : ((((q_in_frame >> 6) * pd.n_frames + frame) << 6) | (q_in_frame & 63u));
}

RT_DEV f3 hit_normal(const InstanceRec &in, uint32_t prim, float bu, float bv)
{
    const float b0 = 1.0f - bu - bv;
    const TriRec nr = in.normals[prim];
    f3 n = mk3(nr.a.x, nr.a.y, nr.a.z) * b0;
    n = n + mk3(nr.a.w, nr.b.x, nr.b.y) * bu;
    n = n + mk3(nr.b.z, nr.b.w, nr.c.x) * bv;
    return n;
}

template <class IO>
RT_DEV f3 directional_light(const PipeDev &pd, IO &io, f3 P, f3 N, uint32_t depth)
{
    const rt_directional_light_params &dl = pd.pfc.directionalLight;
    const f3 L = normalize(mk3(-dl.forwardDir.x, -dl.forwardDir.y, -dl.forwardDir.z));
    const float NoL = saturate(dot(N, L));
    const float vis = io.shadow(0, P, L, RAY_EPSILON, RAY_MAX_T, depth, NoL > 0.0f);
    return mk3(dl.color.x, dl.color.y, dl.color.z) * dl.color.w * NoL * vis;
}

template <class IO>
RT_DEV f3 point_light(const PipeDev &pd, IO &io, f3 P, f3 N, uint32_t depth)
{
    const rt_point_light_params &pl = pd.pfc.pointLight;
    const f3 path = mk3(pl.worldPos.x, pl.worldPos.y, pl.worldPos.z) - P;
    const float dist = length(path);
    const f3 L = normalize(path);
    const float NoL = saturate(dot(N, L));
    const float vis = io.shadow(1, P, L, RAY_EPSILON, dist - RAY_EPSILON, depth, NoL > 0.0f);
    const float falloff = 1.0f / (2.0f * HLSL_PI * dist * dist);
    return mk3(pl.color.x, pl.color.y, pl.color.z) * pl.color.w * NoL * vis * falloff;
}

template <class IO>
RT_DEV f3 ambient_occlusion(const PipeDev &pd, IO &io, f3 P, f3 N, uint32_t pix)
{
    float visibility = 0.0f;
    uint32_t seed = io.pixel_seed(pix);
    for (int i = 0; i < 4; ++i) {
        f3 dir; float NoL, pdf;
        if (pd.pfc.options.cosineHemisphereSampling) {
            dir = cos_hemisphere(seed, N);
            NoL = saturate(dot(N, dir));
            pdf = NoL / HLSL_PI;
        } else {
            dir = uniform_hemisphere(seed, N);
            NoL = saturate(dot(N, dir));
            pdf = 1.0f / (2.0f * HLSL_PI);
        }
        visibility += io.shadow(i, P, dir, RAY_EPSILON, 10.0f, 1u, true) * NoL / pdf;
    }
    const float r = visibility / 4.0f;
    return mk3(r, r, r);
}

template <class IO>
RT_DEV bool black_lobe(const IO &io, const rt_material_params &mp, uint32_t seed, uint32_t depth)
{
    if (!io.secondary_is_black(depth)) return false;
    if (!(mp.roughness >= -0.15f && mp.roughness <= 1.6f)) return false;
    return next_rand(seed) > 0.0f;
}

template <class IO>
RT_DEV f3 shade(const PipeDev &pd, IO &io, const rt_material_params &mp, f3 P, f3 N, f3 D, uint32_t depth, uint32_t pix)
{
    const rt_debug_options &opt = pd.pfc.options;
    if (opt.showAmbientOcclusionOnly) return ambient_occlusion(pd, io, P, N, pix);

    uint32_t seed = io.pixel_seed(pix);

    f3 direct = mk3(0.0f, 0.0f, 0.0f);
    if (opt.debug == 2) {
        if (next_rand(seed) < 0.5f) direct = direct + directional_light(pd, io, P, N, depth) * 2.0f;
        else direct = direct + point_light(pd, io, P, N, depth) * 2.0f;
    } else {
        direct = direct + directional_light(pd, io, P, N, depth);
        direct = direct + point_light(pd, io, P, N, depth);
    }

    f3 indirect = mk3(0.0f, 0.0f, 0.0f);
    if (depth < 1 && !opt.noIndirectDiffuse) {
        f3 color = mk3(0.0f, 0.0f, 0.0f);
        if (opt.cosineHemisphereSampling) {
            const f3 dir = cos_hemisphere(seed, N);
            color = color + io.secondary(0, P, dir, RAY_EPSILON, depth) * HLSL_PI;
        } else {
            const f3 dir = uniform_hemisphere(seed, N);
            const float NoL = saturate(dot(N, dir));
            const float pdf = 1.0f / (2.0f * HLSL_PI);
            color = color + io.secondary(0, P, dir, RAY_EPSILON, depth) * NoL / pdf;
        }
        indirect = indirect + color / 1.0f;
    }

    const f3 diffuse = (direct + indirect) / HLSL_PI;

    f3 fresnel = mk3(0.0f, 0.0f, 0.0f);
    f3 specular = mk3(0.0f, 0.0f, 0.0f);
    if (mp.type == 1u || mp.type == 2u) {
        if (mp.reflectivity > 0.001f) {
            if (black_lobe(io, mp, seed, depth)) {
            } else {
                const float exponent = exp_det((1.0f - mp.roughness) * 12.0f);
                float pdf, brdf;
                const f3 mirror = reflect(D, N);
                const f3 dir = phong_lobe(seed, mirror, exponent, pdf, brdf);
                const f3 refl = io.secondary(1, P, dir, RAY_EPSILON, depth);
                specular = specular + refl * brdf / pdf;
            }
            fresnel = fresnel_schlick(D, N, mk3(mp.specular.x, mp.specular.y, mp.specular.z));
        }
    }

    const f3 albedo = mk3(mp.albedo.x, mp.albedo.y, mp.albedo.z);
    if (depth == 0) {
        if (opt.showIndirectDiffuseOnly) return albedo * indirect / HLSL_PI;
        else if (opt.showIndirectSpecularOnly) return specular * mp.reflectivity * fresnel;
        else if (opt.showFresnelTerm) return fresnel;
        else if (opt.showGBufferAlbedoOnly) return albedo;
        else if (opt.showDirectLightingOnly) return albedo * direct / HLSL_PI;
    }
    f3 r = mk3(mp.emissive.x, mp.emissive.y, mp.emissive.z) * mp.emissive.w;
    r = r + albedo * diffuse;
    r = r + specular * mp.reflectivity * fresnel;
    return r;
}

template <class IO>
RT_DEV f3 shade_aov(const PipeDev &pd, IO &io, const rt_material_params &mp, f3 P, f3 N, f3 D, uint32_t depth, uint32_t pix,
                    f3 &aov_direct, f3 &aov_indirect)
{
    uint32_t seed = io.pixel_seed(pix);
    f3 direct = mk3(0.0f, 0.0f, 0.0f);
    direct = direct + directional_light(pd, io, P, N, depth);
    direct = direct + point_light(pd, io, P, N, depth);
    f3 fresnel = mk3(0.0f, 0.0f, 0.0f);
    f3 specular = mk3(0.0f, 0.0f, 0.0f);
    if (mp.type == 1u || mp.type == 2u) {
        if (mp.reflectivity > 0.001f) {
            if (black_lobe(io, mp, seed, depth)) {
            } else {
                const float exponent = exp_det((1.0f - mp.roughness) * 12.0f);
                float pdf, brdf;
                const f3 mirror = reflect(D, N);
                const f3 dir = phong_lobe(seed, mirror, exponent, pdf, brdf);
                const f3 refl = io.secondary(1, P, dir, RAY_EPSILON, depth);
                specular = specular + refl * brdf / pdf;
            }
            fresnel = fresnel_schlick(D, N, mk3(mp.specular.x, mp.specular.y, mp.specular.z));
        }
    }
    const f3 albedo = mk3(mp.albedo.x, mp.albedo.y, mp.albedo.z);
    const f3 dl = albedo * direct / HLSL_PI;
    const f3 is = specular * mp.reflectivity * fresnel;
    if (depth == 0) { aov_direct = dl; aov_indirect = is; }
    return dl + is;
}

struct Shaded { f3 color, aov_direct, aov_indirect; };

template <class IO>
RT_DEV Shaded closest_hit_aov(const PipeDev &pd, IO &io, const RayD &r, float t, float u, float v, uint32_t prim, uint32_t inst,
                              uint32_t depth, uint32_t pix)
{
    const InstanceRec &in = pd.sc.inst[inst];
    const f3 N = normalize(hit_normal(in, prim, u, v));
    const f3 P = r.o + r.d * t;
    const rt_material_params mp = pd.mats[min(inst, pd.nmats - 1u)];
    Shaded s;
    s.aov_direct = mk3(0.0f, 0.0f, 0.0f);
    s.aov_indirect = mk3(0.0f, 0.0f, 0.0f);
    if (pd.kind == RT_PIPELINE_REALTIME) s.color = shade_aov(pd, io, mp, P, N, r.d, depth, pix, s.aov_direct, s.aov_indirect);
    else s.color = shade(pd, io, mp, P, N, r.d, depth, pix);
    return s;
}

template <class IO>
RT_DEV f3 closest_hit(const PipeDev &pd, IO &io, const RayD &r, float t, float u, float v, uint32_t prim, uint32_t inst,
                      uint32_t depth, uint32_t pix)
{
    return closest_hit_aov(pd, io, r, t, u, v, prim, inst, depth, pix).color;
}

RT_DEV void store_ray(float4 *O, float4 *D, size_t slot, f3 o, float tmin, f3 d, float tmax)
{
    O[slot] = make_float4(o.x, o.y, o.z, tmin);
    D[slot] = make_float4(d.x, d.y, d.z, tmax);
}
RT_DEV void store_invalid(float4 *O, float4 *D, size_t slot)
{
    O[slot] = make_float4(0.0f, 0.0f, 0.0f, 0.0f);
    D[slot] = make_float4(0.0f, 0.0f, 0.0f, -1.0f);
}
RT_DEV RayD load_ray(const float4 *O, const float4 *D, size_t slot)
{
    const float4 a = O[slot], b = D[slot];
    RayD r;
    r.o = mk3(a.x, a.y, a.z); r.tmin = a.w;
    r.d = mk3(b.x, b.y, b.z); r.tmax = b.w;
    return r;
}


struct EmitIO {
    const PipeDev &pd;
    int L;
    uint32_t idx, q;
    uint32_t frame;
    uint32_t shadow_mask, skip_mask, sec_mask;
    f3 shadow_origin;
    RT_DEV EmitIO(const PipeDev &p, int level, uint32_t i, uint32_t qq, uint32_t f) : pd(p), L(level), idx(i), q(qq), frame(f), shadow_mask(0), skip_mask(0), sec_mask(0)
    {
        shadow_origin = mk3(0.0f, 0.0f, 0.0f);
    }
    RT_DEV uint32_t pixel_seed(uint32_t pix) const { return init_rand(pix, pd.pfc.cameraParams.frameCount); }
    RT_DEV bool secondary_is_black(uint32_t depth) const { return depth >= pd.max_rad || L >= MAXD; }
    RT_DEV float shadow(int s, f3 o, f3 d, float tmin, float tmax, uint32_t depth, bool matters)
    {
        if (depth >= pd.max_shadow) return 1.0f;
        const bool skipped = !matters && pd.skip_unlit;
        shadow_mask |= 1u << s;
        if (skipped) skip_mask |= 1u << s;
        if (pd.shadow_compact) {
            shadow_origin = o;
            return 1.0f;
        }
        if (skipped) store_ray(pd.sh_O, pd.sh_D, sh_ray(pd, L, idx, (uint32_t)s), mk3(0.0f, 0.0f, 0.0f), 0.0f, mk3(0.0f, 0.0f, 0.0f), RT_TMAX_SKIPPED);
        else store_ray(pd.sh_O, pd.sh_D, sh_ray(pd, L, idx, (uint32_t)s), o, tmin, d, tmax);
        return 1.0f;
    }
    RT_DEV void finish_shadows(uint32_t shadow_slots) const
    {
        if ((uint32_t)L >= pd.sh_levels) return;
        if (pd.shadow_compact) {
            pd.sh_hits[pd.sh_cbase[L] + idx] = make_float4(shadow_origin.x, shadow_origin.y, shadow_origin.z, __uint_as_float(shadow_mask | (skip_mask << 2) | (frame << 8)));
            return;
        }
        for (uint32_t s = 0; s < shadow_slots; s++)
            if (!(shadow_mask & (1u << s))) store_invalid(pd.sh_O, pd.sh_D, sh_ray(pd, L, idx, s));
    }
    RT_DEV f3 secondary(int w, f3 o, f3 d, float tmin, uint32_t depth)
    {
        if (depth >= pd.max_rad || L >= MAXD) return mk3(0.0f, 0.0f, 0.0f);
        const size_t slot = L == 0 ? (size_t)w * pd.lv[1].rstride + idx : idx;
        store_ray(pd.lv[L + 1].O, pd.lv[L + 1].D, slot, o, tmin, d, RAY_MAX_T);
        pd.lv[L + 1].pix[slot] = q;
        sec_mask |= 1u << w;
        return mk3(0.0f, 0.0f, 0.0f);
    }
};

template <int L, int MAXL>
struct ResolveIO {
    const PipeDev &pd;
    uint32_t idx, pix;
    uint32_t seed0;
    RT_DEV ResolveIO(const PipeDev &p, uint32_t i, uint32_t px) : pd(p), idx(i), pix(px), seed0(init_rand(px, p.pfc.cameraParams.frameCount)) {}
    RT_DEV ResolveIO(const PipeDev &p, uint32_t i, uint32_t px, uint32_t seed) : pd(p), idx(i), pix(px), seed0(seed) {}
    RT_DEV uint32_t pixel_seed(uint32_t) const { return seed0; }
    RT_DEV bool secondary_is_black(uint32_t depth) const { return L >= MAXL || depth >= pd.max_rad; }
    RT_DEV float shadow(int s, f3, f3, float, float, uint32_t depth, bool matters)
    {
        if (depth >= pd.max_shadow) return 1.0f;
        if (!matters && pd.skip_unlit) return 1.0f;
        return shadow_bit(pd, sh_ray(pd, L, idx, (uint32_t)s)) ? 1.0f : 0.0f;
    }
    RT_DEV f3 secondary(int w, f3 o, f3 d, float tmin, uint32_t depth)
    {
        if constexpr (L >= MAXL) {
            return mk3(0.0f, 0.0f, 0.0f);
        } else {
            if (depth >= pd.max_rad) return mk3(0.0f, 0.0f, 0.0f);
            const size_t slot = L == 0 ? (size_t)w * pd.lv[1].rstride + idx : idx;
            const float4 h = pd.lv[L + 1].hit[slot];
            if (h.x == HIT_MISS) return sample_environment(pd, d);
            if (h.x == HIT_UNTRACED) return mk3(0.0f, 0.0f, 0.0f);
            RayD r;
            r.o = o; r.tmin = tmin; r.d = d; r.tmax = RAY_MAX_T;
            ResolveIO<L + 1, MAXL> io(pd, pd.lv[L + 1].slot_j[slot], pix, seed0);
            return closest_hit(pd, io, r, h.x, h.y, h.z, __float_as_uint(h.w), pd.lv[L + 1].inst[slot], depth + 1u, pix);
        }
    }
};

struct LevelResolveIO {
    const PipeDev &pd;
    int L;
    uint32_t idx;
    RT_DEV LevelResolveIO(const PipeDev &p, int level, uint32_t i) : pd(p), L(level), idx(i) {}
    RT_DEV uint32_t pixel_seed(uint32_t pix) const { return init_rand(pix, pd.pfc.cameraParams.frameCount); }
    RT_DEV bool secondary_is_black(uint32_t depth) const { return depth >= pd.max_rad || L >= MAXD; }
    RT_DEV float shadow(int s, f3, f3, float, float, uint32_t depth, bool matters)
    {
        if (depth >= pd.max_shadow) return 1.0f;
        if (!matters && pd.skip_unlit) return 1.0f;
        return shadow_bit(pd, sh_ray(pd, L, idx, (uint32_t)s)) ? 1.0f : 0.0f;
    }
    RT_DEV f3 secondary(int w, f3, f3 d, float, uint32_t depth)
    {
        if (depth >= pd.max_rad || L >= MAXD) return mk3(0.0f, 0.0f, 0.0f);
        const size_t slot = L == 0 ? (size_t)w * pd.lv[1].rstride + idx : idx;
        const float4 h = pd.lv[L + 1].hit[slot];
        if (h.x == HIT_MISS) return sample_environment(pd, d);
        if (h.x == HIT_UNTRACED) return mk3(0.0f, 0.0f, 0.0f);
        const float4 c = pd.lv[L + 1].color[slot];
        return mk3(c.x, c.y, c.z);
    }
};

}
```

dxrexperiments_amd/csrc/rt_trace_wave.h:

```cpp
#pragma once

#include "rt_trace_device.h"

namespace rtd {

typedef float v4f __attribute__((ext_vector_type(4)));
typedef const __attribute__((address_space(1))) v4f *gptr4;

RT_DEV v4f ldg16(const void *base, size_t byte_off)
{
    return *(gptr4)((const char *)base + byte_off);
}

#define RT_TMAX_SKIPPED  (-2.0f)
#define RT_NODE_EMPTY    0x7FFFFFFE
#define RT_NODE_SENTINEL 0x7FFFFFFF

#ifndef RT_REFILL_LANES
#define RT_REFILL_LANES 16
#endif
#ifndef RT_REFILL_PRIO
#define RT_REFILL_PRIO 3
#endif
#ifndef RT_LEAF_PRIO
#define RT_LEAF_PRIO 1
#endif
#ifndef RT_LOAD_PRIO
#define RT_LOAD_PRIO 2
#endif
#ifndef RT_POOL_CHUNK
#define RT_POOL_CHUNK 64u
#endif
#ifndef RT_POOL_CHUNK_SETS
#define RT_POOL_CHUNK_SETS 128u
#endif

#ifndef RT_POOL_CHUNK_SETS_ANYHIT
#define RT_POOL_CHUNK_SETS_ANYHIT 256u
#endif
#ifndef RT_POOL_GROUPS
#define RT_POOL_GROUPS 32u
#endif
#define RT_POOL_STRIDE 32u
#ifndef RT_SENTINEL_INLINE
#define RT_SENTINEL_INLINE 1
#endif
#ifndef RT_POOL_XCD
#define RT_POOL_XCD 1
#endif
#ifndef RT_REFILL_RAYS_PER_PASS
#define RT_REFILL_RAYS_PER_PASS 28u
#endif
#ifndef RT_REFILL_ENTER_TESTS
#define RT_REFILL_ENTER_TESTS 32
#endif
#ifndef RT_REFILL_STOP_TESTS
#define RT_REFILL_STOP_TESTS 32
#endif
#ifndef RT_REFILL_ENTER_TESTS_SETS
#define RT_REFILL_ENTER_TESTS_SETS 48
#endif
#ifndef RT_REFILL_STOP_TESTS_SETS
#define RT_REFILL_STOP_TESTS_SETS 24
#endif
#ifndef RT_REFILL_TESTS_TWO_LEVEL
#define RT_REFILL_TESTS_TWO_LEVEL 1
#endif
#ifndef RT_REFILL_TESTS
#define RT_REFILL_TESTS 1
#endif
#ifndef RT_EXIT_K
#define RT_EXIT_K 1
#endif

}
#include "rt_wide_step.h"
namespace rtd {

RT_DEV uint32_t distinct_node_lines(int node, bool from_global)
{
    unsigned long long todo = __ballot(from_global);
    uint32_t n = 0;
    while (todo) {
        const int l = __builtin_ctzll(todo);
        const int v = __builtin_amdgcn_readlane(node, l);
        todo &= ~__ballot(from_global && node == v);
        n++;
    }
    return n;
}

RT_DEV bool node_is_internal(int node) { return node >= 0 && node < RT_NODE_EMPTY; }

template <class S, class = void> struct src_has_cache { static constexpr bool value = false; };
template <class S> struct src_has_cache<S, decltype((void)&S::has_first_candidates)> { static constexpr bool value = true; };

RT_DEV unsigned long long lanemask_lt()
{
    const uint32_t lane = threadIdx.x & 63u;
    return (1ull << lane) - 1ull;
}

template <class S> RT_DEV auto load_ray_of(const S &src, uint32_t i, RayD &r, uint32_t &ticket, int) -> decltype(src.load(i, r, ticket)) { return src.load(i, r, ticket); }
template <class S> RT_DEV bool load_ray_of(const S &src, uint32_t i, RayD &r, uint32_t &ticket, long) { ticket = i; return src.load(i, r); }

#define RT_WALK_WORDS 11
template <int STACK, int BLOCK, bool TWO_LEVEL, uint32_t CHUNK, bool ANYHIT = false, bool COUNT = false, bool NO_DEEP = false, bool REFS = false, class Src, class Sink>
RT_DEV void trace_wave(const SceneDev &sc, const Src &src, const Sink &sink, uint32_t *pool, int *smem, uint32_t *traced_counter,
                       unsigned long long *walk = nullptr)
{
    uint32_t rf_loaded = 0, rf_passes = 0;
    uint32_t n_traced = 0;
    uint32_t n_skipped = 0;
    uint32_t wk_glob = 0, wk_top = 0, wk_tri = 0, wk_inst = 0, wk_lines = 0;
    uint32_t wk_ray0 = 0;
    unsigned long long wk_longest = 0;
    uint32_t wv_steps = 0, wv_leaf = 0, wv_tri = 0;
    uint32_t wk_node_lines = 0;
    const uint32_t total = src.count();
    const uint32_t flags = src.flags();
    const bool first = ANYHIT ? true : (flags & RT_RAY_FLAG_ACCEPT_FIRST_HIT_AND_END_SEARCH) != 0;
    const bool cull = (flags & RT_RAY_FLAG_CULL_BACK_FACING_TRIANGLES) != 0;
    LaneStack<STACK, BLOCK> st;
    st.lds = smem + threadIdx.x;
    st.threads = gridDim.x * BLOCK;
    st.deep = sc.deep_stack && !NO_DEEP ? sc.deep_stack + (size_t)blockIdx.x * BLOCK + threadIdx.x : nullptr;

    const InstanceRec *in0 = sc.inst;
    const WNode *blas_nodes0 = TWO_LEVEL ? nullptr : in0->wide;
    const TriRec *tris0 = TWO_LEVEL ? nullptr : in0->tris;
    int *topl = smem + STACK * BLOCK;
    if (sc.top_n != 0) {
        const int *src_top = (const int *)(TWO_LEVEL ? sc.tlas_wide : blas_nodes0);
        for (uint32_t i = threadIdx.x; i < sc.top_n * RT_TOP_WORDS; i += BLOCK) topl[i] = src_top[(i / RT_TOP_WORDS) * (uint32_t)(sizeof(WNode) / 4) + i % RT_TOP_WORDS];
    }
    const int *const top_cur = topl;
    if (sc.top_n != 0) __syncthreads();
    const int root0 = TWO_LEVEL ? sc.tlas_root_code : in0->root_code;
    uint32_t top_lim = sc.top_n;

    bool alive = false;
    bool exhausted = false;
    uint32_t chunk_next = 0, chunk_end = 0;
    const uint32_t n_waves = gridDim.x * (BLOCK / 64);
    uint32_t next_chunk = blockIdx.x * (BLOCK / 64) + threadIdx.x / 64;
    const uint32_t n_groups = gridDim.x < RT_POOL_GROUPS ? gridDim.x : RT_POOL_GROUPS;
    const uint32_t pool_group = blockIdx.x % n_groups;
#if RT_POOL_XCD
    uint32_t xcd_steal = 0;
#endif
    uint32_t idx = 0;
    RayD r;
    RayInv wri;
    HitD best;
    int node = RT_NODE_EMPTY;
    int sp = 0;
    ObjRay cur;
    const WNode *nodes = TWO_LEVEL ? sc.tlas_wide : blas_nodes0;
    const InstanceRec *in = in0;
    const TriRec *tris = tris0;
    uint32_t ii = 0;
    bool in_blas = !TWO_LEVEL;
    r.o = mk3(0, 0, 0); r.d = mk3(0, 0, 1); r.tmin = 0; r.tmax = 0;
    wri = make_inv(r.o, r.d);
    cur.o = r.o; cur.d = r.d; cur.ri = wri;
    best = make_miss(r);

    for (;;) {
        constexpr bool REFILL_TESTS = src_has_cache<Src>::value && ANYHIT && !COUNT && (!TWO_LEVEL || RT_REFILL_TESTS_TWO_LEVEL) && RT_REFILL_TESTS;
        unsigned long long idle = __ballot(!alive);
        int n_idle = __popcll(idle);
        if (REFILL_TESTS) rf_passes++;
        const bool mostly_answered = REFILL_TESTS && rf_loaded >= RT_REFILL_RAYS_PER_PASS * rf_passes && rf_loaded >= 64u;
        const int REFILL_ENTER = mostly_answered ? (CHUNK > 64u ? RT_REFILL_ENTER_TESTS_SETS : RT_REFILL_ENTER_TESTS) : RT_REFILL_LANES;
        const int REFILL_STOP = mostly_answered ? (CHUNK > 64u ? RT_REFILL_STOP_TESTS_SETS : RT_REFILL_STOP_TESTS) : RT_REFILL_LANES;
        for (int refill_round = 0; !exhausted && n_idle >= (refill_round == 0 ? REFILL_ENTER : REFILL_STOP) && (refill_round == 0 || REFILL_TESTS); refill_round++) {
#if RT_REFILL_PRIO
            __builtin_amdgcn_s_setprio(RT_REFILL_PRIO);
#endif
            if (chunk_next >= chunk_end) {
                uint32_t cidx;
#if RT_POOL_XCD
                if (ANYHIT && pool && n_groups == RT_POOL_GROUPS) {
                    const uint32_t chunks = (total + CHUNK - 1u) / CHUNK, per = (chunks + 7u) / 8u;
                    cidx = 0x4000000u;
                    while (xcd_steal < 8u) {
                        const uint32_t x = (pool_group + xcd_steal) & 7u;
                        const uint32_t g = x + (pool_group & ~7u);
                        uint32_t k = 0;
                        if ((threadIdx.x & 63u) == 0u) k = atomicAdd(&pool[g * RT_POOL_STRIDE], 1u);
                        k = (uint32_t)__builtin_amdgcn_readfirstlane((int)k);
                        const uint32_t c = x * per + (pool_group >> 3) + k * (RT_POOL_GROUPS / 8u);
                        if (c < (x + 1u) * per && c < chunks) { cidx = c; break; }
                        xcd_steal++;
                    }
                } else
#endif
                if (pool) {
                    uint32_t k = 0;
                    if ((threadIdx.x & 63u) == 0u) k = atomicAdd(&pool[pool_group * RT_POOL_STRIDE], 1u);
                    k = (uint32_t)__builtin_amdgcn_readfirstlane((int)k);
                    cidx = pool_group + k * n_groups;
                } else {
                    cidx = next_chunk;
                    next_chunk += n_waves;
                }
                const uint32_t base = cidx < 0x4000000u ? cidx * CHUNK : total;
                chunk_next = base;
                chunk_end = base + CHUNK < total ? base + CHUNK : total;
                if (base >= total) { exhausted = true; chunk_end = chunk_next; }
            }
            const uint32_t avail = chunk_end - chunk_next;
            const uint32_t rank = (uint32_t)__popcll(idle & lanemask_lt());
            bool started = false, skipped = false;
            if (!alive && rank < avail) {
                const uint32_t my = chunk_next + rank;
                const bool traced = load_ray_of(src, my, r, idx, 0);
                best = make_miss(r);
                if (traced && r.tmax > r.tmin && sc.n_inst != 0) {
                    wri = make_inv(r.o, r.d);
                    cur.o = r.o; cur.d = r.d; cur.ri = wri;
                    node = root0;
                    sp = 0;
                    if (TWO_LEVEL) { nodes = sc.tlas_wide; in_blas = false; top_lim = sc.top_n; }
                    bool occluded_at_once = false;
                    if constexpr (REFILL_TESTS) {
                        uint32_t slot, ci;
                        const uint32_t ct = src.template cached_leaf<TWO_LEVEL>(idx, r, slot, ci);
                        st.lds[(STACK - 1) * BLOCK] = (int)slot;
                        if (ct != RT_NO_HIT && (!TWO_LEVEL || (ci < sc.n_inst && ct < sc.inst[ci].n_recs))) {
                            const InstanceRec *cin = TWO_LEVEL ? sc.inst + ci : in0;
                            const ObjRay orr = TWO_LEVEL ? to_object(*cin, r) : cur;
                            const char *tp = (const char *)((TWO_LEVEL ? cin->tris : tris0) + ct);
                            const v4f a = ldg16(tp, 0), b = ldg16(tp, 16), c = ldg16(tp, 32);
                            HitD found = best;
                            if (accept_candidate<REFS ? 1 : 0>(*cin, TWO_LEVEL ? ci : 0u, __float_as_uint(c.y), mk3(a.x, a.y, a.z), mk3(a.w, b.x, b.y), mk3(b.z, b.w, c.x), r, wri, orr, cull, found,
                                                               REFS ? __float_as_uint(c.z) : 0u, ct)) {
                                sink.store(idx, found, true);
                                occluded_at_once = true;
                            }
                        }
                    } else
                    if constexpr (src_has_cache<Src>::value && ANYHIT && !COUNT) {
                        uint32_t slot, ci;
                        const uint32_t ct = src.template cached_leaf<TWO_LEVEL>(idx, r, slot, ci);
                        st.lds[(STACK - 1) * BLOCK] = (int)slot;
                        if (ct != RT_NO_HIT && (!TWO_LEVEL || (ci < sc.n_inst && ct < sc.inst[ci].n_recs))) {
                            st.lds[0] = root0;
                            sp = 1;
                            if (TWO_LEVEL) {
                                ii = ci;
                                in = sc.inst + ii;
                                cur = to_object(*in, r);
                                nodes = in->wide;
                                tris = in->tris;
                                in_blas = true;
                                top_lim = 0;
                                st.lds[BLOCK] = RT_NODE_SENTINEL;
                                sp = 2;
                            }
                            node = ~(int)(ct << 3);
                        }
                    }
                    alive = !occluded_at_once;
                    started = true;
                    if (COUNT) wk_ray0 = wk_glob + wk_top;
                } else {
                    if (ANYHIT && r.tmax == RT_TMAX_SKIPPED) skipped = true;
                    sink.store(idx, best, traced);
                }
            }
            n_traced += (uint32_t)__popcll(__ballot(started));
            if (REFILL_TESTS) rf_loaded += (uint32_t)__popcll(__ballot(started));
            if (ANYHIT) n_skipped += (uint32_t)__popcll(__ballot(skipped));
            chunk_next += (uint32_t)n_idle < avail ? (uint32_t)n_idle : avail;
#if RT_REFILL_PRIO
            __builtin_amdgcn_s_setprio(0);
#endif
            idle = __ballot(!alive);
            n_idle = __popcll(idle);
        }
        if (__ballot(alive) == 0ull) {
            if (exhausted) break;
            continue;
        }

#if RT_EXIT_K > 0
        const int n_alive = __popcll(__ballot(alive));
#endif
        while (alive && node_is_internal(node) && sp <= STACK - (RT_WIDE - 1)) {
            if (COUNT) {
                if ((uint32_t)node < top_lim) wk_top++; else wk_glob++;
                const uint32_t dl = distinct_node_lines(node, !((uint32_t)node < top_lim));
                if ((threadIdx.x & 63u) == (uint32_t)__builtin_ctzll(__builtin_amdgcn_read_exec())) { wk_lines += (RT_WIDE == 8 ? 2u : 1u) * dl; wk_node_lines += (RT_WIDE == 8 ? 2u : 1u) * dl; wv_steps++; }
            }
            wide_step<false, ANYHIT>(nodes, top_cur, top_lim, cur.ri, r.tmin, ANYHIT ? r.tmax : best.t, st, node, sp);
#if RT_SENTINEL_INLINE
            if (TWO_LEVEL && node == RT_NODE_SENTINEL) {
                in_blas = false;
                nodes = sc.tlas_wide;
                top_lim = sc.top_n;
                cur.o = r.o; cur.d = r.d; cur.ri = wri;
                if (sp > 0) { sp--; node = st.lds[sp * BLOCK]; }
                else node = RT_NODE_EMPTY;
            }
#endif
#if RT_EXIT_K > 0
            const int walking = __popcll(__ballot(alive && node_is_internal(node)));
            if (walking * RT_EXIT_K < n_alive - walking) break;
#endif
        }
        bool gave_up = NO_DEEP && alive && node_is_internal(node) && sp > STACK - (RT_WIDE - 1);
        if constexpr (!NO_DEEP) {
            while (alive && node_is_internal(node) && sp > STACK - (RT_WIDE - 1)) {
                if (COUNT) {
                    if ((uint32_t)node < top_lim) wk_top++; else wk_glob++;
                    const uint32_t dl = distinct_node_lines(node, !((uint32_t)node < top_lim));
                    if ((threadIdx.x & 63u) == (uint32_t)__builtin_ctzll(__builtin_amdgcn_read_exec())) { wk_lines += (RT_WIDE == 8 ? 2u : 1u) * dl; wk_node_lines += (RT_WIDE == 8 ? 2u : 1u) * dl; wv_steps++; }
                }
                wide_step<true, ANYHIT>(nodes, top_cur, top_lim, cur.ri, r.tmin, ANYHIT ? r.tmax : best.t, st, node, sp);
            }
        }

#if RT_LEAF_PRIO
        __builtin_amdgcn_s_setprio(RT_LEAF_PRIO);
#endif
        if (alive && !node_is_internal(node)) {
            bool pop = true;
            if (COUNT && (threadIdx.x & 63u) == (uint32_t)__builtin_ctzll(__builtin_amdgcn_read_exec())) wv_leaf++;
            if (node == RT_NODE_EMPTY) {
                sink.store(idx, ANYHIT ? make_miss(r) : best, true);
                alive = false;
                pop = false;
                if (COUNT) { const unsigned long long w = ((unsigned long long)(wk_glob + wk_top - wk_ray0) << 32) | idx; wk_longest = w > wk_longest ? w : wk_longest; }
            } else if (TWO_LEVEL && node == RT_NODE_SENTINEL) {
                in_blas = false;
                nodes = sc.tlas_wide;
                top_lim = sc.top_n;
                cur.o = r.o; cur.d = r.d; cur.ri = wri;
            } else if (TWO_LEVEL && !in_blas) {
                ii = (uint32_t)~node;
                in = sc.inst + ii;
                if (COUNT) wk_inst++;
                bool enter = true;
                if (sc.n_inst == 1) {
                    float e;
                    enter = slab_hit(wri, in->wlo[0], in->whi[0], in->wlo[1], in->whi[1], in->wlo[2], in->whi[2], r.tmin, best.t, e);
                }
                if (NO_DEEP && enter && sp >= STACK) {
                    gave_up = true;
                    pop = false;
                } else if (enter) {
                    cur = to_object(*in, r);
                    nodes = in->wide;
                    tris = in->tris;
                    in_blas = true;
                    top_lim = 0;
                    if constexpr (NO_DEEP) st.lds[sp * BLOCK] = RT_NODE_SENTINEL;
                    else st.write(sp, RT_NODE_SENTINEL);
                    sp++;
                    node = in->root_code;
                    pop = false;
                }
            } else {
                const uint32_t code = (uint32_t)~node;
                const uint32_t first_tri = code >> 3, cnt = (code & 7u) + 1u;
                for (uint32_t k = 0; k < cnt; k++) {
                    if (COUNT) {
                        wk_tri++;
                        const uint32_t by = (first_tri + k) * 48u;
                        wk_lines += 1u + ((by & 63u) > 16u ? 1u : 0u);
                        if ((threadIdx.x & 63u) == (uint32_t)__builtin_ctzll(__builtin_amdgcn_read_exec())) wv_tri++;
                    }
                    const char *tp = (const char *)(tris + first_tri + k);
                    const v4f a = ldg16(tp, 0), b = ldg16(tp, 16), c = ldg16(tp, 32);
                    const uint32_t prim = __float_as_uint(c.y);
                    HitD found = ANYHIT ? make_miss(r) : best;
                    const bool accepted = accept_candidate<REFS ? 1 : 0>(*in, ii, prim, mk3(a.x, a.y, a.z), mk3(a.w, b.x, b.y), mk3(b.z, b.w, c.x), r, wri, cur, cull, found,
                                                                         REFS ? __float_as_uint(c.z) : 0u, first_tri + k);
                    if (!ANYHIT) best = found;
                    if (accepted && first) {
                        if constexpr (src_has_cache<Src>::value && ANYHIT && !COUNT) src.template remember<TWO_LEVEL>((uint32_t)st.lds[(STACK - 1) * BLOCK], first_tri + k, ii);
                        sink.store(idx, found, true);
                        alive = false;
                        pop = false;
                        if (COUNT) { const unsigned long long w = ((unsigned long long)(wk_glob + wk_top - wk_ray0) << 32) | idx; wk_longest = w > wk_longest ? w : wk_longest; }
                        break;
                    }
                }
            }
            if (pop) {
                if (sp > 0) {
                    sp--;
                    if constexpr (NO_DEEP) node = st.lds[sp * BLOCK];
                    else node = st.read(sp);
                }
                else node = RT_NODE_EMPTY;
            }
        }
        if constexpr (NO_DEEP) {
            if (gave_up) { src.overflow(idx); alive = false; }
        }
#if RT_LEAF_PRIO
        __builtin_amdgcn_s_setprio(0);
#endif
    }
    if (COUNT && walk) {
        const unsigned long long w9[10] = {(threadIdx.x & 63u) == 0u ? n_traced : 0u, wk_glob, wk_top, wk_tri, wk_inst, wk_lines, wv_steps, wv_leaf, wv_tri, wk_node_lines};
        for (int k = 0; k < 10; k++) {
            unsigned long long v = w9[k];
            for (int o = 32; o > 0; o >>= 1) v += (unsigned long long)__shfl_xor((long long)v, o, 64);
            if ((threadIdx.x & 63u) == 0u && v) atomicAdd(&walk[k < 6 ? k : k + 1], v);
        }
        atomicMax(&walk[6], wk_longest);
    }
    if (traced_counter) {
        if ((threadIdx.x & 63u) == 0u && n_traced) atomicAdd(traced_counter, n_traced);
        if (ANYHIT && (threadIdx.x & 63u) == 0u && n_skipped) atomicAdd(traced_counter + 1, n_skipped);
    }
}

}
```

Baseline: 11320.

## Fuse last-level secondary trace with shadow-hit emission, skipping compaction and shade pass

For the deepest bounce level, a fused secondary trace kernel writes the shadow-hit entries (hit point, light mask, frame index) straight from the traversal sink and tallies hits with wave ballots. This removes the compact-level kernel, the host counter readback and sync, and the separate shade-emit launch for that level. The shadow queue is generalized into segments so the fused level's uncompacted slots map correctly, and the resolve path indexes fused slots directly. The cost is shadow work over uncompacted slots, with miss slots producing no-op entries, plus added complexity in segment ticket arithmetic.

```diff
diff --git a/dxrexperiments_amd/csrc/rt_pipeline.hip b/dxrexperiments_amd/csrc/rt_pipeline.hip
--- a/dxrexperiments_amd/csrc/rt_pipeline.hip
+++ b/dxrexperiments_amd/csrc/rt_pipeline.hip
@@ -163,7 +163,7 @@
     const RayD r = L == 0 ? primary_ray(pd, px, py) : load_ray(pd.lv[L].O, pd.lv[L].D, slot);
     const float4 h = pd.lv[L].hit[slot];
     if (!PRIMARY && !emit_next && pd.shadow_compact && !pd.skip_unlit) {
-        const f3 P = r.o + r.d * h.x;
+        const f3 P = hit_point(r.o, r.d, h.x);
         uint32_t mask = 3u;
         if (pd.kind != RT_PIPELINE_REALTIME && pd.pfc.options.debug == 2) {
             uint32_t seed = init_rand(px + py * pd.width, pd.pfc.cameraParams.frameCount);
@@ -225,22 +225,54 @@
         inst1[sl] = h.inst;
     }
 };
-
+struct FusedOut {
+    float4 *entries;
+    const uint32_t *pix;
+    uint32_t *nhit;
+    uint32_t n_frames, frames_magic;
+};
+struct FusedSecondarySink {
+    QueueSrc q;
+    float4 *hit1;
+    uint32_t *inst1;
+    FusedOut fo;
+    static constexpr bool tallies_hits = true;
+    RT_DEV void add_hits(uint32_t n) const { atomicAdd(fo.nhit, n); }
+    RT_DEV void store(uint32_t i, const HitD &h, bool traced, const RayD &r) const
+    {
+        const size_t sl = q.slot(i);
+        const bool hit = h.inst != RT_NO_HIT;
+        hit1[sl] = make_float4(hit ? h.t : (traced ? HIT_MISS : HIT_UNTRACED), h.u, h.v, __uint_as_float(h.prim));
+        inst1[sl] = h.inst;
+        __builtin_amdgcn_sched_barrier(0);
+        const f3 P = hit_point(r.o, r.d, h.t);
+        uint32_t bits = hit ? 3u : 0u;
+        if (fo.pix && hit) bits |= slot_frame_magic(fo.n_frames, fo.frames_magic, fo.pix[sl]) << 8;
+        float zero;
+        asm volatile("v_mov_b32 %0, 0" : "=v"(zero));
+        fo.entries[sl] = make_float4(hit ? P.x : zero, hit ? P.y : zero, hit ? P.z : zero, hit ? __uint_as_float(bits) : zero);
+    }
+};
+
+constexpr int SH_SEGS = MAXD + 2;
 struct ShadowQueue {
     const float4 *hits, *O, *D;
     uint32_t *vis;
     const uint32_t *nhit;
     uint32_t log2, fl;
-    uint32_t lv_first, lv_count;
-    uint32_t cbase[MAXD + 1], hstride[MAXD + 1];
+    uint32_t seg_first, seg_count;
+    uint32_t seg_counter;
+    uint32_t seg_split, split_adj;
+    uint32_t cbase[SH_SEGS], hstride[SH_SEGS];
     LightRays lights;
     const LightRays *frame_lights;
     ShadowCacheDev cache;
+    RT_DEV uint32_t seg_n(uint32_t k) const { return nhit[(seg_counter >> (4u * k)) & 15u]; }
     RT_DEV uint32_t count() const
     {
         uint32_t b = 0;
 #pragma unroll
-        for (uint32_t k = 0; k <= (uint32_t)MAXD; k++) if (k >= lv_first && k < lv_first + lv_count) b += (nhit[k] + 63u) & ~63u;
+        for (uint32_t k = 0; k < (uint32_t)SH_SEGS; k++) if (k >= seg_first && k < seg_first + seg_count) b += (seg_n(k) + 63u) & ~63u;
         return b << log2;
     }
     RT_DEV uint32_t flags() const { return fl; }
@@ -249,23 +281,25 @@
 struct ShadowSrcN : ShadowQueue {
     RT_DEV bool load(uint32_t i, RayD &r, uint32_t &ticket) const
     {
-        uint32_t n = 0, R = 0, cb = 0, hs = 0, before = 0;
+        uint32_t n = 0, cb = 0, hs = 0, tb = 0, before = 0;
         ticket = 0;
 #pragma unroll
-        for (uint32_t k = 0; k <= (uint32_t)MAXD; k++) {
-            if (k >= lv_first && k < lv_first + lv_count) {
-                const uint32_t nk = nhit[k], Rk = (nk + 63u) & ~63u, start = before;
-                before += Rk << log2;
+        for (uint32_t k = 0; k < (uint32_t)SH_SEGS; k++) {
+            if (k >= seg_first && k < seg_first + seg_count) {
+                const uint32_t nk = seg_n(k), start = before;
+                before += ((nk + 63u) & ~63u) << log2;
                 const bool here = i >= start;
-                n = here ? nk : n; R = here ? Rk : R; cb = here ? cbase[k] : cb; hs = here ? hstride[k] : hs;
+                n = here ? nk : n; cb = here ? cbase[k] : cb; hs = here ? hstride[k] : hs;
+                tb = here ? (cbase[k] << log2) - (k == seg_split ? split_adj : 0u) : tb;
                 if (here) ticket = start;
             }
         }
+        const uint32_t R = (n + 63u) & ~63u;
         const uint32_t local = i - ticket;
         uint32_t b = local >= R ? 1u : 0u;
         if (log2 > 1u) { b += local >= 2u * R ? 1u : 0u; b += local >= 3u * R ? 1u : 0u; }
         const uint32_t j = local - b * R;
-        ticket = (cb << log2) + b * hs + j;
+        ticket = tb + b * hs + j;
         r.o = mk3(0.0f, 0.0f, 0.0f);
         r.d = mk3(0.0f, 0.0f, 0.0f);
         r.tmin = 0.0f;
@@ -275,7 +309,7 @@
             const v4f a = ldg16(hits, (size_t)(cb + j) * 16);
             const uint32_t bits = __float_as_uint(a.w);
             r.o = mk3(a.x, a.y, a.z);
-            if (!((bits >> b) & 1u)) return false;
+            if (!((bits >> b) & 1u)) { ticket = RT_NO_HIT; return false; }
             if ((bits >> (2u + b)) & 1u) { r.tmax = RT_TMAX_SKIPPED; return false; }
             r.tmin = RAY_EPSILON;
             const LightRays *per_frame = BATCH ? frame_lights : nullptr;
@@ -381,6 +415,13 @@
 {
     __shared__ int smem[(RT_ROWS(STACK) + RT_TOP_ROWS(PBLOCK)) * PBLOCK];
     SecondarySink sink = {src, hit1, inst1};
+    trace_wave<RT_ROWS(STACK), PBLOCK, TWO_LEVEL, (!TWO_LEVEL && RT_ROWS(STACK) == RT_LDS_STACK_ROWS_SETS) ? RT_POOL_CHUNK_SETS : RT_POOL_CHUNK, false, false, false, RT_REFS(STACK)>(sc, src, sink, pool, smem, stat);
+}
+template <int STACK, bool TWO_LEVEL>
+__global__ void __launch_bounds__(PBLOCK) RT_WAVES_PER_EU k_trace_secondary_fused(SceneDev sc, QueueSrc src, float4 *hit1, uint32_t *inst1, uint32_t *pool, uint32_t *stat, FusedOut fo)
+{
+    __shared__ int smem[(RT_ROWS(STACK) + RT_TOP_ROWS(PBLOCK)) * PBLOCK];
+    FusedSecondarySink sink = {src, hit1, inst1, fo};
     trace_wave<RT_ROWS(STACK), PBLOCK, TWO_LEVEL, (!TWO_LEVEL && RT_ROWS(STACK) == RT_LDS_STACK_ROWS_SETS) ? RT_POOL_CHUNK_SETS : RT_POOL_CHUNK, false, false, false, RT_REFS(STACK)>(sc, src, sink, pool, smem, stat);
 }
 
@@ -484,9 +525,17 @@
 {
     PipeDev pd = pd_arg;
     const int L = LC >= 0 ? LC : level;
-    const uint32_t idx = blockIdx.x * PBLOCK + threadIdx.x;
-    if (idx >= pd.counters[C_NHIT + L]) return;
-    const uint32_t slot = pd.lv[L].jlist[idx];
+    __builtin_assume(L >= 1);
+    uint32_t idx = blockIdx.x * PBLOCK + threadIdx.x;
+    uint32_t slot;
+    if (RT_FUSE_LAST_LEVEL && (uint32_t)L == pd.fused_level) {
+        if (idx >= pd.counters[C_NHIT + L - 1]) return;
+        slot = idx;
+        if (!(pd.lv[L].hit[slot].x >= 0.0f)) return;
+    } else {
+        if (idx >= pd.counters[C_NHIT + L]) return;
+        slot = pd.lv[L].jlist[idx];
+    }
     const uint32_t q = pd.lv[L].pix[slot];
     uint32_t px, py, ql = q;
     if (BATCH) pd.pfc = pd.pfcs[slot_frame(pd, q, ql)];
@@ -561,6 +610,35 @@
 }
 
 namespace {
+
+ShadowQueue shadow_queue(const PipeDev &pd, uint32_t flags, const LightRays &lights)
+{
+    ShadowQueue sq;
+    memset(&sq, 0, sizeof sq);
+    sq.hits = pd.sh_hits; sq.O = pd.sh_O; sq.D = pd.sh_D; sq.vis = pd.sh_vis;
+    sq.nhit = &pd.counters[C_NHIT];
+    sq.log2 = pd.sh_log2; sq.fl = flags;
+    sq.lights = lights;
+    sq.frame_lights = pd.n_frames > 1u ? pd.frame_lights : nullptr;
+    sq.seg_split = (uint32_t)SH_SEGS;
+    uint32_t s = 0;
+    for (uint32_t l = 0; l <= (uint32_t)MAXD; l++) {
+        const bool fused = RT_FUSE_LAST_LEVEL && l != 0u && l == pd.fused_level;
+        for (uint32_t b = 0; b < (fused && l == 1u ? 2u : 1u); b++, s++) {
+            sq.cbase[s] = pd.sh_cbase[l] + b * pd.lv[1].rstride;
+            sq.hstride[s] = pd.lv[l].hstride;
+            sq.seg_counter |= (fused ? l - 1u : l) << (4u * s);
+            if (b) { sq.seg_split = s; sq.split_adj = pd.lv[1].rstride * ((1u << pd.sh_log2) - 1u); }
+        }
+    }
+    return sq;
+}
+void select_levels(ShadowQueue &sq, const PipeDev &pd, uint32_t first, uint32_t count)
+{
+    auto seg_of = [&](uint32_t l) { return l + (RT_FUSE_LAST_LEVEL && pd.fused_level == 1u && l > 1u ? 1u : 0u); };
+    sq.seg_first = seg_of(first);
+    sq.seg_count = seg_of(first + count) - sq.seg_first;
+}
 
 template <int STACK, bool TWO_LEVEL>
 int launch_frame(rt_pipeline *p, PipeDev &pd, uint32_t shadow_slots, bool counted)
@@ -578,8 +656,9 @@
     const uint32_t any = RT_RAY_FLAG_ACCEPT_FIRST_HIT_AND_END_SEARCH | RT_RAY_FLAG_SKIP_CLOSEST_HIT_SHADER;
     size_t hits_l = cap, slots = cap;
     size_t sh_total = 0;
-    auto size_next = [&](uint32_t l, bool casts_shadows, bool spawns) -> int {
-        if (counted) {
+    auto size_next = [&](uint32_t l, bool casts_shadows, bool spawns, bool fused = false) -> int {
+        if (fused) hits_l = slots;
+        else if (counted) {
             HIP_TRY(hipMemcpyAsync(ctx->pinned, &pd.counters[C_NHIT + l], 4, hipMemcpyDeviceToHost, st));
             HIP_TRY(hipStreamSynchronize(st));
             hits_l = round64((size_t)ctx->pinned[0]);
@@ -622,11 +701,23 @@
     const LightRays lr = light_rays(pd);
     for (uint32_t l = 1; l <= levels; l++) {
         const QueueSrc rays = {pd.lv[l].O, pd.lv[l].D, &pd.counters[C_NHIT + l - 1], pd.lv[1].rstride, l == 1 ? 2u : 1u, RT_RAY_FLAG_NONE};
+        const bool casts_shadows = l < pd.sh_levels, spawns = l < levels;
+#if RT_FUSE_LAST_LEVEL
+        if (l == pd.fused_level) {
+            const size_t ray_slots = slots;
+            RT_TRY(size_next(l, true, false, true));
+            const FusedOut fo = {pd.sh_hits + pd.sh_cbase[l], B ? pd.lv[l].pix : nullptr, &pd.counters[C_NHIT + l], pd.n_frames,
+                                 (uint32_t)(0x100000000ull / (pd.n_frames ? pd.n_frames : 1u)) + 1u};
+            k_trace_secondary_fused<STACK, TWO_LEVEL><<<rt_persistent_grid(ctx, k_trace_secondary_fused<STACK, TWO_LEVEL>, PBLOCK, ray_slots), PBLOCK, 0, st>>>(
+                pd.sc, rays, pd.lv[l].hit, pd.lv[l].inst, pd.pools + (size_t)l * RT_POOL_GROUPS * RT_POOL_STRIDE, &pd.counters[C_SECONDARY], fo);
+            if (T) { record(ev[3 + 2 * (l - 1)], st); record(ev[4 + 2 * (l - 1)], st); }
+            continue;
+        }
+#endif
         k_trace_secondary<STACK, TWO_LEVEL><<<rt_persistent_grid(ctx, k_trace_secondary<STACK, TWO_LEVEL>, PBLOCK, slots), PBLOCK, 0, st>>>(
             pd.sc, rays, pd.lv[l].hit, pd.lv[l].inst, pd.pools + (size_t)l * RT_POOL_GROUPS * RT_POOL_STRIDE, &pd.counters[C_SECONDARY]);
         k_compact_level<<<(unsigned)((slots + CTILES * CBLOCK - 1) / (CTILES * CBLOCK)), CBLOCK, 0, st>>>(pd, (int)l);
         if (T) record(ev[3 + 2 * (l - 1)], st);
-        const bool casts_shadows = l < pd.sh_levels, spawns = l < levels;
         RT_TRY(size_next(l, casts_shadows, spawns));
         if (casts_shadows || spawns) {
             if (B) k_shade_emit<false, true><<<blocks(hits_l), PBLOCK, 0, st>>>(pd, (int)l, 2u, spawns ? 1u : 0u);
@@ -635,15 +726,8 @@
         if (T) record(ev[4 + 2 * (l - 1)], st);
     }
     {
-        ShadowQueue sq;
-        memset(&sq, 0, sizeof sq);
-        sq.hits = pd.sh_hits; sq.O = pd.sh_O; sq.D = pd.sh_D; sq.vis = pd.sh_vis;
-        sq.nhit = &pd.counters[C_NHIT];
-        sq.log2 = pd.sh_log2; sq.fl = any;
-        sq.lv_first = 0; sq.lv_count = pd.sh_levels;
-        for (int k = 0; k <= MAXD; k++) { sq.cbase[k] = pd.sh_cbase[k]; sq.hstride[k] = pd.lv[k].hstride; }
-        sq.lights = lr;
-        sq.frame_lights = B ? pd.frame_lights : nullptr;
+        ShadowQueue sq = shadow_queue(pd, any, lr);
+        select_levels(sq, pd, 0, pd.sh_levels);
         sq.cache = p->shadow_cache_dev;
         sq.cache.jlist0 = pd.lv[0].jlist;
         sq.cache.hstride0 = pd.lv[0].hstride;
@@ -694,22 +778,15 @@
     k_walk_primary<TWO_LEVEL><<<rt_persistent_grid(ctx, k_walk_primary<TWO_LEVEL>, PBLOCK, cap), PBLOCK, 0, st>>>(pd, w + RT_WALK_WORDS * RT_STAGE_PRIMARY);
     const unsigned gq = rt_persistent_grid(ctx, k_walk_queue<TWO_LEVEL>, PBLOCK, (size_t)cap * 2);
     const unsigned gs = rt_persistent_grid(ctx, k_walk_shadow<TWO_LEVEL>, PBLOCK, (size_t)cap * 2);
-    ShadowQueue sq;
-    memset(&sq, 0, sizeof sq);
-    sq.hits = pd.sh_hits; sq.O = pd.sh_O; sq.D = pd.sh_D; sq.vis = pd.sh_vis;
-    sq.nhit = &pd.counters[C_NHIT];
-    sq.log2 = pd.sh_log2; sq.fl = any;
-    sq.lights = light_rays(pd);
-    sq.frame_lights = pd.n_frames > 1u ? pd.frame_lights : nullptr;
-    for (int k = 0; k <= MAXD; k++) { sq.cbase[k] = pd.sh_cbase[k]; sq.hstride[k] = pd.lv[k].hstride; }
-    sq.lv_first = 0; sq.lv_count = 1;
+    ShadowQueue sq = shadow_queue(pd, any, light_rays(pd));
+    select_levels(sq, pd, 0, 1);
     k_walk_shadow<TWO_LEVEL><<<gs, PBLOCK, 0, st>>>(pd.sc, sq, w + RT_WALK_WORDS * RT_STAGE_SHADOW0);
     const uint32_t levels = pd.max_rad < (uint32_t)MAXD ? pd.max_rad : (uint32_t)MAXD;
     for (uint32_t l = 1; l <= levels; l++)
         k_walk_queue<TWO_LEVEL><<<gq, PBLOCK, 0, st>>>(pd.sc, QueueSrc{pd.lv[l].O, pd.lv[l].D, &pd.counters[C_NHIT + l - 1], pd.lv[1].rstride, l == 1 ? 2u : 1u, RT_RAY_FLAG_NONE},
                                                        w + RT_WALK_WORDS * RT_STAGE_SECONDARY);
     if (pd.sh_levels > 1u) {
-        sq.lv_first = 1; sq.lv_count = pd.sh_levels - 1u;
+        select_levels(sq, pd, 1, pd.sh_levels - 1u);
         k_walk_shadow<TWO_LEVEL><<<gs, PBLOCK, 0, st>>>(pd.sc, sq, w + RT_WALK_WORDS * RT_STAGE_SHADOW1);
     }
     HIP_TRY(hipGetLastError());
@@ -738,14 +815,8 @@
     const uint32_t any = RT_RAY_FLAG_ACCEPT_FIRST_HIT_AND_END_SEARCH | RT_RAY_FLAG_SKIP_CLOSEST_HIT_SHADER;
     k_count_primary<<<blocks(cap), PBLOCK, 0, st>>>(pd, w + 3 * RT_STAGE_PRIMARY);
     ShadowSrcN<true> sq;
-    memset(&sq, 0, sizeof sq);
-    sq.hits = pd.sh_hits; sq.O = pd.sh_O; sq.D = pd.sh_D; sq.vis = pd.sh_vis;
-    sq.nhit = &pd.counters[C_NHIT];
-    sq.log2 = pd.sh_log2; sq.fl = any;
-    sq.lights = light_rays(pd);
-    sq.frame_lights = pd.n_frames > 1u ? pd.frame_lights : nullptr;
-    for (int k = 0; k <= MAXD; k++) { sq.cbase[k] = pd.sh_cbase[k]; sq.hstride[k] = pd.lv[k].hstride; }
-    sq.lv_first = 0; sq.lv_count = 1;
+    static_cast<ShadowQueue &>(sq) = shadow_queue(pd, any, light_rays(pd));
+    select_levels(sq, pd, 0, 1);
     k_count_queue<<<blocks((size_t)pd.lv[0].hstride << pd.sh_log2), PBLOCK, 0, st>>>(pd.sc, sq, w + 3 * RT_STAGE_SHADOW0);
     const uint32_t levels = pd.max_rad < (uint32_t)MAXD ? pd.max_rad : (uint32_t)MAXD;
     size_t deeper = 0;
@@ -757,7 +828,7 @@
         if (l < pd.sh_levels) deeper += pd.lv[l].hstride;
     }
     if (pd.sh_levels > 1u) {
-        sq.lv_first = 1; sq.lv_count = pd.sh_levels - 1u;
+        select_levels(sq, pd, 1, pd.sh_levels - 1u);
         k_count_queue<<<blocks(deeper << pd.sh_log2), PBLOCK, 0, st>>>(pd.sc, sq, w + 3 * RT_STAGE_SHADOW1);
     }
     HIP_TRY(hipGetLastError());
diff --git a/dxrexperiments_amd/csrc/rt_pipeline_dev.h b/dxrexperiments_amd/csrc/rt_pipeline_dev.h
--- a/dxrexperiments_amd/csrc/rt_pipeline_dev.h
+++ b/dxrexperiments_amd/csrc/rt_pipeline_dev.h
@@ -12,6 +12,10 @@
 #define RT_SHADOW_UNORDERED 1
 #endif
 static_assert(RT_SHADOW_UNORDERED != 0, "the shadow stage counts skipped slots in the ANYHIT walk only");
+
+#ifndef RT_FUSE_LAST_LEVEL
+#define RT_FUSE_LAST_LEVEL 1
+#endif
 
 #define RAY_MAX_T 1.0e+38f
 #define RAY_EPSILON 0.0001f
@@ -96,6 +100,7 @@
     uint32_t sh_log2;
     uint32_t sh_levels;
     uint32_t sh_cbase[MAXD + 1];
+    uint32_t fused_level;
     uint32_t *pools;
     LevelDev lv[MAXD + 1];
 };
diff --git a/dxrexperiments_amd/csrc/rt_pipeline_render.hip b/dxrexperiments_amd/csrc/rt_pipeline_render.hip
--- a/dxrexperiments_amd/csrc/rt_pipeline_render.hip
+++ b/dxrexperiments_amd/csrc/rt_pipeline_render.hip
@@ -266,6 +266,12 @@
     pd.accum_f16 = p->accum_f16;
     pd.skip_unlit = p->skip_unlit;
     pd.kind = p->kind;
+    pd.fused_level = 0;
+    if (RT_FUSE_LAST_LEVEL && levels_now >= 1u && levels_now < pd.sh_levels && !ao_view && !p->skip_unlit) {
+        bool one_light_view = false;
+        for (uint32_t f = 0; f < n_frames; f++) one_light_view = one_light_view || (p->kind != RT_PIPELINE_REALTIME && frames[f].options.debug == 2);
+        if (!one_light_view) pd.fused_level = levels_now;
+    }
     {
         rt_pipeline::PrimaryMode &pm = p->primary_mode;
         if (pm.gen != p->scene->generation) { pm.gen = p->scene->generation; pm.samples = 0; pm.persistent = false; pm.in_flight = false; }
diff --git a/dxrexperiments_amd/csrc/rt_shade.h b/dxrexperiments_amd/csrc/rt_shade.h
--- a/dxrexperiments_amd/csrc/rt_shade.h
+++ b/dxrexperiments_amd/csrc/rt_shade.h
@@ -112,6 +112,11 @@
     q_in_frame = (tile << 6) | (q & 63u);
     return f;
 }
+RT_DEV uint32_t slot_frame_magic(uint32_t n_frames, uint32_t frames_magic, uint32_t q)
+{
+    const uint32_t c = q >> 6;
+    return c - __umulhi(c, frames_magic) * n_frames;
+}
 RT_DEV uint32_t frame_slot(const PipeDev &pd, uint32_t frame, uint32_t q_in_frame)
 {
     return pd.n_frames <= 1u ? q_in_frame : ((((q_in_frame >> 6) * pd.n_frames + frame) << 6) | (q_in_frame & 63u));
@@ -278,13 +283,15 @@
 
 struct Shaded { f3 color, aov_direct, aov_indirect; };
 
+RT_DEV f3 hit_point(const f3 &o, const f3 &d, float t) { return o + d * t; }
+
 template <class IO>
 RT_DEV Shaded closest_hit_aov(const PipeDev &pd, IO &io, const RayD &r, float t, float u, float v, uint32_t prim, uint32_t inst,
                               uint32_t depth, uint32_t pix)
 {
     const InstanceRec &in = pd.sc.inst[inst];
     const f3 N = normalize(hit_normal(in, prim, u, v));
-    const f3 P = r.o + r.d * t;
+    const f3 P = hit_point(r.o, r.d, t);
     const rt_material_params mp = pd.mats[min(inst, pd.nmats - 1u)];
     Shaded s;
     s.aov_direct = mk3(0.0f, 0.0f, 0.0f);
@@ -396,7 +403,7 @@
             if (h.x == HIT_UNTRACED) return mk3(0.0f, 0.0f, 0.0f);
             RayD r;
             r.o = o; r.tmin = tmin; r.d = d; r.tmax = RAY_MAX_T;
-            ResolveIO<L + 1, MAXL> io(pd, pd.lv[L + 1].slot_j[slot], pix, seed0);
+            ResolveIO<L + 1, MAXL> io(pd, RT_FUSE_LAST_LEVEL && pd.fused_level == (uint32_t)(L + 1) ? (uint32_t)slot : pd.lv[L + 1].slot_j[slot], pix, seed0);
             return closest_hit(pd, io, r, h.x, h.y, h.z, __float_as_uint(h.w), pd.lv[L + 1].inst[slot], depth + 1u, pix);
         }
     }
diff --git a/dxrexperiments_amd/csrc/rt_trace_wave.h b/dxrexperiments_amd/csrc/rt_trace_wave.h
--- a/dxrexperiments_amd/csrc/rt_trace_wave.h
+++ b/dxrexperiments_amd/csrc/rt_trace_wave.h
@@ -103,6 +103,10 @@
 
 template <class S> RT_DEV auto load_ray_of(const S &src, uint32_t i, RayD &r, uint32_t &ticket, int) -> decltype(src.load(i, r, ticket)) { return src.load(i, r, ticket); }
 template <class S> RT_DEV bool load_ray_of(const S &src, uint32_t i, RayD &r, uint32_t &ticket, long) { ticket = i; return src.load(i, r); }
+template <class S> RT_DEV auto store_hit_of(const S &sink, uint32_t t, const HitD &h, bool traced, const RayD &r, int) -> decltype(sink.store(t, h, traced, r)) { sink.store(t, h, traced, r); }
+template <class S> RT_DEV void store_hit_of(const S &sink, uint32_t t, const HitD &h, bool traced, const RayD &, long) { sink.store(t, h, traced); }
+template <class S, class = void> struct sink_tallies_hits { static constexpr bool value = false; };
+template <class S> struct sink_tallies_hits<S, decltype((void)&S::tallies_hits)> { static constexpr bool value = true; };
 
 #define RT_WALK_WORDS 11
 template <int STACK, int BLOCK, bool TWO_LEVEL, uint32_t CHUNK, bool ANYHIT = false, bool COUNT = false, bool NO_DEEP = false, bool REFS = false, class Src, class Sink>
@@ -112,6 +116,8 @@
     uint32_t rf_loaded = 0, rf_passes = 0;
     uint32_t n_traced = 0;
     uint32_t n_skipped = 0;
+    constexpr bool TALLY = sink_tallies_hits<Sink>::value && !ANYHIT;
+    uint32_t n_hits = 0;
     uint32_t wk_glob = 0, wk_top = 0, wk_tri = 0, wk_inst = 0, wk_lines = 0;
     uint32_t wk_ray0 = 0;
     unsigned long long wk_longest = 0;
@@ -119,7 +125,7 @@
     uint32_t wk_node_lines = 0;
     const uint32_t total = src.count();
     const uint32_t flags = src.flags();
-    const bool first = ANYHIT ? true : (flags & RT_RAY_FLAG_ACCEPT_FIRST_HIT_AND_END_SEARCH) != 0;
+    const bool first = ANYHIT ? true : TALLY ? false : (flags & RT_RAY_FLAG_ACCEPT_FIRST_HIT_AND_END_SEARCH) != 0;
     const bool cull = (flags & RT_RAY_FLAG_CULL_BACK_FACING_TRIANGLES) != 0;
     LaneStack<STACK, BLOCK> st;
     st.lds = smem + threadIdx.x;
@@ -211,7 +217,8 @@
                 if (base >= total) { exhausted = true; chunk_end = chunk_next; }
             }
             const uint32_t avail = chunk_end - chunk_next;
-            const uint32_t rank = (uint32_t)__popcll(idle & lanemask_lt());
+            const uint32_t rank = TALLY ? __builtin_amdgcn_mbcnt_hi((uint32_t)(idle >> 32), __builtin_amdgcn_mbcnt_lo((uint32_t)idle, 0u))
+                                        : (uint32_t)__popcll(idle & lanemask_lt());
             bool started = false, skipped = false;
             if (!alive && rank < avail) {
                 const uint32_t my = chunk_next + rank;
@@ -236,7 +243,7 @@
                             HitD found = best;
                             if (accept_candidate<REFS ? 1 : 0>(*cin, TWO_LEVEL ? ci : 0u, __float_as_uint(c.y), mk3(a.x, a.y, a.z), mk3(a.w, b.x, b.y), mk3(b.z, b.w, c.x), r, wri, orr, cull, found,
                                                                REFS ? __float_as_uint(c.z) : 0u, ct)) {
-                                sink.store(idx, found, true);
+                                store_hit_of(sink, idx, found, true, r, 0);
                                 occluded_at_once = true;
                             }
                         }
@@ -267,7 +274,7 @@
                     if (COUNT) wk_ray0 = wk_glob + wk_top;
                 } else {
                     if (ANYHIT && r.tmax == RT_TMAX_SKIPPED) skipped = true;
-                    sink.store(idx, best, traced);
+                    store_hit_of(sink, idx, best, traced, r, 0);
                 }
             }
             n_traced += (uint32_t)__popcll(__ballot(started));
@@ -325,11 +332,18 @@
 #if RT_LEAF_PRIO
         __builtin_amdgcn_s_setprio(RT_LEAF_PRIO);
 #endif
+        bool ended_hit = false;
         if (alive && !node_is_internal(node)) {
             bool pop = true;
             if (COUNT && (threadIdx.x & 63u) == (uint32_t)__builtin_ctzll(__builtin_amdgcn_read_exec())) wv_leaf++;
             if (node == RT_NODE_EMPTY) {
-                sink.store(idx, ANYHIT ? make_miss(r) : best, true);
+                if constexpr (TWO_LEVEL) store_hit_of(sink, idx, ANYHIT ? make_miss(r) : best, true, r, 0);
+                else {
+                    RayD rs;
+                    rs.o = cur.o; rs.d = cur.d; rs.tmin = r.tmin; rs.tmax = r.tmax;
+                    store_hit_of(sink, idx, ANYHIT ? make_miss(r) : best, true, rs, 0);
+                }
+                if (TALLY) ended_hit = best.inst != RT_NO_HIT;
                 alive = false;
                 pop = false;
                 if (COUNT) { const unsigned long long w = ((unsigned long long)(wk_glob + wk_top - wk_ray0) << 32) | idx; wk_longest = w > wk_longest ? w : wk_longest; }
@@ -381,7 +395,7 @@
                     if (!ANYHIT) best = found;
                     if (accepted && first) {
                         if constexpr (src_has_cache<Src>::value && ANYHIT && !COUNT) src.template remember<TWO_LEVEL>((uint32_t)st.lds[(STACK - 1) * BLOCK], first_tri + k, ii);
-                        sink.store(idx, found, true);
+                        store_hit_of(sink, idx, found, true, r, 0);
                         alive = false;
                         pop = false;
                         if (COUNT) { const unsigned long long w = ((unsigned long long)(wk_glob + wk_top - wk_ray0) << 32) | idx; wk_longest = w > wk_longest ? w : wk_longest; }
@@ -404,7 +418,9 @@
 #if RT_LEAF_PRIO
         __builtin_amdgcn_s_setprio(0);
 #endif
+        if (TALLY) n_hits += (uint32_t)__popcll(__ballot(ended_hit));
     }
+    if constexpr (TALLY) { if ((threadIdx.x & 63u) == 0u && n_hits) sink.add_hits(n_hits); }
     if (COUNT && walk) {
         const unsigned long long w9[10] = {(threadIdx.x & 63u) == 0u ? n_traced : 0u, wk_glob, wk_top, wk_tri, wk_inst, wk_lines, wv_steps, wv_leaf, wv_tri, wk_node_lines};
         for (int k = 0; k < 10; k++) {
```

Measured after the change: 11090. -2.0%, worse.
